# Jimmy2027/MoPoE-MIMIC

Measured on AMD Instinct MI355X. Metric: samples/sec, higher is better.
Workload: dtype f32; 1 GPU; BASELINE config c2: MoPoE joint-ELBO train step, 3 modalities (PA+Lateral+text) 128x128, class_dim 128, DIM_img 64, DIM_text 128, vocab 3517, batch 64/GPU, fp32 (storage, accumulation and every product; where the launch plan says so the fp32 products are formed on the bf16 matrix pipe from exact three-way splits of both operands -- closer to fp64 than the fp32 MFMA, tests: test_f32_products_on_the; global_batch=64, parallelism=dp1, hip_graph=True, cross_rank_elbo=mean

## Files before the change

### include/mopoe_hip.h

```cpp
#ifndef MOPOE_HIP_H
#define MOPOE_HIP_H

#include <stddef.h>
#include <stdint.h>

#ifdef __cplusplus
extern "C" {
#endif

#define MOPOE_ABI_VERSION 23

#define MOPOE_OK 0
#define MOPOE_ERR_ARG (-1)
#define MOPOE_ERR_LAUNCH (-2)
#define MOPOE_ERR_DEVICE (-3)

int mopoe_abi_version(void);
const char* mopoe_last_error(void);

typedef struct {
  int32_t N;
  int32_t Hs, Ws;
  int32_t Hb, Wb;
  int32_t Cin, Cout;
  int32_t kh, kw;
  int32_t sh, sw;
  int32_t ph, pw;
  int32_t transposed;
} mopoe_conv_geom;

typedef struct {
  const double* sums;
  const float* gamma;
  const float* beta;
  const float* rmean;
  const float* rvar;
  double inv_count;
  float eps;
  int32_t C;
  int32_t mode;
} mopoe_bn_ref;

typedef struct {
  const float* mask;
  int32_t kind;
  int32_t rows_per_sample;
} mopoe_mask_ref;

size_t mopoe_conv_workspace_bytes(void);

typedef struct {
  int32_t tile;
  int32_t split;
} mopoe_conv_plan;

int mopoe_conv_fwd(const float* x, const float* wp, const float* bias, float* y,
                   const mopoe_conv_geom* g, const mopoe_bn_ref* bn_in, const mopoe_mask_ref* mask,
                   double* out_stats, const mopoe_conv_plan* plan, void* workspace, size_t workspace_bytes,
                   void* stream);

typedef struct {
  const void* s;
  mopoe_bn_ref bn;
  float a, b;
} mopoe_mix_ref;
int mopoe_conv_fwd_mix(const float* x, const float* wp, const float* bias, float* y, const mopoe_conv_geom* g,
                       const mopoe_bn_ref* bn_in, const mopoe_mask_ref* mask, const mopoe_mix_ref* mix,
                       double* out_stats, const mopoe_conv_plan* plan, void* workspace, size_t workspace_bytes,
                       void* stream);

int mopoe_conv_dgrad(const float* dy, const float* wp, float* dx, const mopoe_conv_geom* g,
                     const mopoe_bn_ref* relu_bn, const float* xin, double* bwd_sums,
                     const mopoe_conv_plan* plan, void* workspace, size_t workspace_bytes, void* stream);

int mopoe_conv_wgrad(const float* x, const float* dy, float* dwp, const mopoe_conv_geom* g,
                     const mopoe_bn_ref* bn_in, int32_t dwp_is_zero, const mopoe_conv_plan* plan, void* stream);

int mopoe_block_out_fwd(const float* s, const float* m, float* out, int64_t rows, int32_t C,
                        const mopoe_bn_ref* bn_s, float a, float b, double* out_stats, void* stream);

int mopoe_bn_relu_apply(const float* x, float* out, int64_t rows, int32_t C, const mopoe_bn_ref* bn, void* stream);

int mopoe_bn_bwd_reduce(const float* g, const float* s, int64_t rows, int32_t C,
                        const mopoe_bn_ref* bn_s, double* sums, void* stream);

int mopoe_block_out_bwd(const float* g, const float* s, float* dm, float* ds, int64_t rows, int32_t C,
                        const mopoe_bn_ref* bn_s, const double* sums, const mopoe_mask_ref* mask,
                        float a, float b, float* dgamma, float* dbeta, float* colsum_dm,
                        float* colsum_ds, void* stream);

int mopoe_bn_bwd_apply(const float* dy, const float* x, const float* add, float* dx, int64_t rows,
                       int32_t C, const mopoe_bn_ref* bn, const double* sums,
                       const mopoe_mask_ref* mask, float* dgamma, float* dbeta, float* colsum_dx,
                       const float* next_s, const mopoe_bn_ref* next_bn, double* next_sums, void* stream);

typedef struct {
  const double* sums;
  float* rmean;
  float* rvar;
  int32_t C;
  int32_t count;
} mopoe_bn_running_desc;
int mopoe_bn_running_update(const mopoe_bn_running_desc* desc, int32_t n, float momentum, void* stream);

int mopoe_colsum(const float* x, float* out, int64_t rows, int32_t C, int32_t out_is_zero, void* stream);

int mopoe_latent_fwd(const float* const mu_in[3], const float* const lv_in[3], const float* eps,
                     int32_t B, int32_t D, const int32_t* row_start, const float* w, float norm,
                     float* mus, float* lvs, float* joint_mu, float* joint_lv, float* z, float* klds,
                     float* joint_div, double* kl_ws, void* stream);

int mopoe_latent_bwd(const float* const mu_in[3], const float* const lv_in[3], const float* eps,
                     int32_t B, int32_t D, const int32_t* row_start, const float* w, float norm,
                     const float* g_mus, const float* g_lvs, const float* g_joint_mu,
                     const float* g_joint_lv, const float* g_z, const float* g_klds,
                     const float* g_joint_div, float* const d_mu_in[3], float* const d_lv_in[3],
                     void* stream);

#define MOPOE_LATENT_MOE 0
#define MOPOE_LATENT_JSD 1
int mopoe_latent_mixture_fwd(int32_t method, const float* const mu_in[3], const float* const lv_in[3],
                             const float* eps, int32_t B, int32_t D, const int32_t* member_row_start,
                             const int32_t* comp_row_start, const float* w, float norm, float* sub_mu,
                             float* sub_lv, float* comp_mu, float* comp_lv, float* joint_mu, float* joint_lv,
                             float* z, float* klds, float* individual_divs, float* joint_div, float* pd_mu,
                             float* pd_lv, double* ws, void* stream);

int mopoe_latent_mixture_bwd(int32_t method, const float* const mu_in[3], const float* const lv_in[3],
                             const float* eps, int32_t B, int32_t D, const int32_t* member_row_start,
                             const int32_t* comp_row_start, const float* w, float norm, const float* g_sub_mu,
                             const float* g_sub_lv, const float* g_comp_mu, const float* g_comp_lv,
                             const float* g_joint_mu, const float* g_joint_lv, const float* g_z,
                             const float* g_klds, const float* g_individual_divs, const float* g_joint_div,
                             const float* g_pd_mu, const float* g_pd_lv, float* const d_mu_in[3],
                             float* const d_lv_in[3], void* stream);

int mopoe_latent_style_fwd(const float* const smu[3], const float* const slv[3], const float* const eps_s[3],
                           const int32_t S[3], int32_t B, int32_t D, const float* z, float norm, float* const zcat[3],
                           float* klds_style, double* ws, void* stream);

int mopoe_latent_style_bwd(const float* const smu[3], const float* const slv[3], const float* const eps_s[3],
                           const int32_t S[3], int32_t B, int32_t D, float norm, const float* const g_zcat[3],
                           const float* g_klds_style, float* const d_smu[3], float* const d_slv[3], float* g_z,
                           void* stream);

int mopoe_laplace_nll_fwd(const float* x_hat, const float* x, int64_t n, float scale, float norm,
                          float* out, double* ws, void* stream);
int mopoe_laplace_nll_bwd(const float* x_hat, const float* x, const float* g, int64_t n, float scale,
                          float norm, float* dx_hat, void* stream);

int mopoe_logsoftmax_fwd(const float* x, float* y, int64_t rows, int32_t V, void* stream);
int mopoe_logsoftmax_bwd(const float* dy, const float* y, float* dx, int64_t rows, int32_t V,
                         void* stream);
int mopoe_token_nll_fwd(const float* logp, const float* ids, int64_t rows, int32_t V, float norm,
                        float* out, double* ws, void* stream);
int mopoe_token_nll_bwd(const float* ids, const float* g, int64_t rows, int32_t V, float norm,
                        float* dlogp, void* stream);

int mopoe_dense_nll_fwd(const float* logp, const float* target, int64_t n, float norm, float* out, double* ws,
                        void* stream);
int mopoe_dense_nll_bwd(const float* target, const float* g, int64_t n, float norm, float* dlogp, void* stream);

int mopoe_laplace_logprob_rows(const float* x_hat, const float* x, int64_t rows, int64_t per_row,
// ... 104 lines not shown
```

### mopoe-mimic_amd/csrc/conv_gemm.hip

```cpp
#include "gemm_common.hpp"

namespace mopoe {

constexpr int BK = 16;
#ifndef TILE_N64_REMAINDER
#define TILE_N64_REMAINDER 64
#endif
#ifndef SPLIT_BLOCKS
#define SPLIT_BLOCKS 256
#endif
#ifndef SPLIT_TARGET
#define SPLIT_TARGET 512
#endif
#ifndef GEMM_8WAVES
#define GEMM_8WAVES 1
#endif
#ifndef PERSIST_BLOCKS
#define PERSIST_BLOCKS 2048
#endif
#ifndef GEMM_MIN_WAVES
#define GEMM_MIN_WAVES 3
#endif
#ifndef GEMM_BK_BIG
#define GEMM_BK_BIG 16
#endif
#ifndef GEMM_LDS_PAD
#define GEMM_LDS_PAD 4
#endif
constexpr int LDS_PAD = GEMM_LDS_PAD;

struct GemmArgs {
  const float* X;
  const float* W;
  float* Y;
  const float* bias;
  int N, Hx, Wx, Hy, Wy, Ck, Cn, Cin_w, Cout_w;
  int kh, kw, sh, sw, ph, pw;
  int form, w_nk;
  int Hq, Wq;
  long rows_per_phase;
  int vecA, vecB;
  mopoe_bn_ref bn_in;
  mopoe_mask_ref mask;
  double* out_stats;
  mopoe_bn_ref relu_bn;
  const float* xin;
  double* bwd_sums;
  unsigned x_bytes, w_bytes;
  int nsplit;
  float* partial;
  int* counters;
  long rows_total;
  int mix;
  float mix_a, mix_b;
  int xcd_remap;
};

__device__ __forceinline__ float epi_round(const GemmArgs&, float x) { return x; }
struct EpiXinRaw { float4 lo, hi; };
constexpr bool EPI_PREFETCH_XIN = false;
__device__ __forceinline__ EpiXinRaw epi_xin_ld(const GemmArgs& a, long yrow, int ncol, bool ok_hi) {
  const float* p = a.xin + yrow * a.Cn + ncol;
  EpiXinRaw r;
  r.lo = *reinterpret_cast<const float4*>(p);
  r.hi = ok_hi ? *reinterpret_cast<const float4*>(p + 4) : make_float4(0.f, 0.f, 0.f, 0.f);
  return r;
}
__device__ __forceinline__ void epi_xin_unpack(const EpiXinRaw& r, float (&xi)[8]) {
  xi[0] = r.lo.x; xi[1] = r.lo.y; xi[2] = r.lo.z; xi[3] = r.lo.w; xi[4] = r.hi.x; xi[5] = r.hi.y; xi[6] = r.hi.z; xi[7] = r.hi.w;
}
__device__ __forceinline__ void epi_store8(const GemmArgs& a, long yrow, int ncol, bool ok_hi, const float (&v)[8]) {
  float* dst = a.Y + yrow * a.Cn + ncol;
  *reinterpret_cast<float4*>(dst) = make_float4(v[0], v[1], v[2], v[3]);
  if (ok_hi) *reinterpret_cast<float4*>(dst + 4) = make_float4(v[4], v[5], v[6], v[7]);
}


__device__ __forceinline__ float4 bld4(__amdgpu_buffer_rsrc_t srd, unsigned byte_off) {
  const u32x4 v = __builtin_amdgcn_raw_buffer_load_b128(srd, byte_off, 0, 0);
  return make_float4(__uint_as_float(v.x), __uint_as_float(v.y), __uint_as_float(v.z), __uint_as_float(v.w));
}

__device__ __forceinline__ float4 bld4s(__amdgpu_buffer_rsrc_t srd, unsigned byte_off, unsigned s_off) {
  const u32x4 v = __builtin_amdgcn_raw_buffer_load_b128(srd, byte_off, s_off, 0);
  return make_float4(__uint_as_float(v.x), __uint_as_float(v.y), __uint_as_float(v.z), __uint_as_float(v.w));
}

__device__ __forceinline__ float4 ld4(const float* p, int nvalid, bool vec) {
  float4 v = make_float4(0.f, 0.f, 0.f, 0.f);
  if (nvalid >= 4 && vec) {
    v = *reinterpret_cast<const float4*>(p);
  } else {
    if (nvalid > 0) v.x = p[0];
    if (nvalid > 1) v.y = p[1];
    if (nvalid > 2) v.z = p[2];
    if (nvalid > 3) v.w = p[3];
  }
  return v;
}

template <int BM, int BN, int WGM, int WGN, int GBK, bool VEC, int SPEC = 0>
__global__ __launch_bounds__(64 * WGM * WGN, (WGM * WGN == 4 ? GEMM_MIN_WAVES : ((BM / WGM) * (BN / WGN) > 64 * 32 ? 2 : 4)))
void gather_gemm_kernel(const GemmArgs a) {
  static_assert(SPEC == 0 || VEC, "specialised loops exist for the vector path only");
  constexpr int NT = 64 * WGM * WGN;
  static_assert(WGM * WGN == 4 || WGM * WGN == 8, "4 or 8 waves per block");
  constexpr int WM = BM / WGM, WN = BN / WGN;
  constexpr int TI = WM / 32, TJ = WN / 32;
  constexpr int A_LD = BM + LDS_PAD, B_LD = BN + LDS_PAD;
  constexpr int KQ = GBK / 4;
  constexpr int RPP = NT / KQ;
  constexpr int A_PER_THR = BM / RPP;
  static_assert(BM % RPP == 0, "A tile rows must be a multiple of the rows covered per pass");
  constexpr int B_PER_THR_NK = (BN + RPP - 1) / RPP;
  constexpr int N4 = BN / 4;
  constexpr int B_PER_THR_KN = (GBK * N4 + NT - 1) / NT;
  constexpr int B_PER_THR = B_PER_THR_NK > B_PER_THR_KN ? B_PER_THR_NK : B_PER_THR_KN;

  constexpr int STG_LD = WN + 4;
  constexpr int A_FLOATS = 2 * GBK * A_LD, B_FLOATS = 2 * GBK * B_LD;
  constexpr int STG_FLOATS = VEC ? (NT / 64) * 32 * STG_LD : 0;
  constexpr int SMEM_FLOATS = (A_FLOATS + B_FLOATS) > STG_FLOATS ? (A_FLOATS + B_FLOATS) : STG_FLOATS;
  __shared__ __attribute__((aligned(16))) float smem[SMEM_FLOATS];
  __shared__ __attribute__((aligned(16))) float bnS[MAX_BN_C];
  __shared__ __attribute__((aligned(16))) float bnT[MAX_BN_C];
  __shared__ __attribute__((aligned(16))) float epi[5][VEC ? BN : 4];
  __shared__ int s_ticket;
  float* const As0 = smem;
  float* const Bs0 = smem + A_FLOATS;
#define AS_(buf, k, r) As0[((buf) * GBK + (k)) * A_LD + (r)]
#define BS_(buf, k, r) Bs0[((buf) * GBK + (k)) * B_LD + (r)]

  const int tid = threadIdx.x;
  const int lane = tid & 63, wave = tid >> 6;
  const int wm = wave / WGN, wn = wave % WGN;
  unsigned lbx = blockIdx.x, lby = blockIdx.y, lbz = blockIdx.z;
  if (a.xcd_remap) {
    const unsigned inner = gridDim.y * gridDim.z;
    const unsigned sw = xcd_swizzle(blockIdx.x + gridDim.x * (blockIdx.y + gridDim.y * blockIdx.z), gridDim.x * inner);
    lbx = sw / inner;
    const unsigned rem = sw - lbx * inner;
    lby = rem % gridDim.y;
    lbz = rem / gridDim.y;
  }
  const int n0 = lby * BN;
  const int phase = lbz / a.nsplit;
  const int split = lbz - phase * a.nsplit;

  const TapWalk tw = tap_walk(a, phase);
  const int nty = tw.nty, ntx = tw.ntx, ky0 = tw.ky0, kx0 = tw.kx0, kstep_y = tw.kstep_y, kstep_x = tw.kstep_x;
  const int dsgn = tw.dsgn, cy = tw.cy, cx = tw.cx, phy = tw.phy, phx = tw.phx;
  const int nkc = (a.Ck + GBK - 1) / GBK;
  const int total_all = nty * ntx * nkc;
// ... 359 lines not shown
  float cbias[TJ], s1[TJ], s2[TJ];
  BnC rbc[TJ];
  unsigned voffB[TJ];
#pragma unroll
  for (int j = 0; j < TJ; ++j) {
    const int n = n0 + wn * WN + j * 32 + l31;
    s1[j] = s2[j] = 0.f;
    cbias[j] = (n < a.Cn && a.bias && !a.partial) ? a.bias[n] : 0.f;
    rbc[j] = BnC{0.f, 0.f, 0.f, 0.f};
    if (n < a.Cn && do_relu_bn && !a.partial) rbc[j] = bn_coef(a.relu_bn, n);
    if (n < a.Cn) voffB[j] = w_nk ? ((unsigned)n * (unsigned)a.Cout_w + (unsigned)lhi * 4u) * 4u
                                  : ((unsigned)lhi * 4u * (unsigned)a.Cout_w + (unsigned)n) * 4u;
    else voffB[j] = OOB;
  }

  const long nMt = (a.rows_per_phase + BM - 1) / BM;
  for (long mt = lbx; mt < nMt; mt += gridDim.x) {
    const long m0 = mt * BM;
    int ry0[TI], rx0[TI], rbase[TI];
    bool rvalid[TI];
#pragma unroll
    for (int i = 0; i < TI; ++i) {
      const long m = m0 + wm * WM + i * 32 + l31;
      rvalid[i] = m < a.rows_per_phase;
      const unsigned mm = rvalid[i] ? (unsigned)m : 0u;
      const int n = (int)(mm / (unsigned)hw);
      const int rem = (int)(mm - (unsigned)n * (unsigned)hw);
      const int qy = rem / a.Wq, qx = rem - qy * a.Wq;
      if (a.form == 0) { ry0[i] = qy * a.sh - a.ph; rx0[i] = qx * a.sw - a.pw; }
      else             { ry0[i] = qy + cy;          rx0[i] = qx + cx; }
      rbase[i] = (n * a.Hx + ry0[i]) * a.Wx + rx0[i];
    }

    int ld_tap = it_beg / nkc;
    int ld_kc = (it_beg - ld_tap * nkc) * KS;
    bool tap_dirty = true;
    unsigned offA[TI], offW = 0;
    bool okA[TI];
    float4 ra[2][TI], rsc[2], rsh[2];
    float rbd[2][TJ][4];
    float4 rb4[2][TJ];
    bool rok[2][TI];

    auto load_step = [&](auto bufc) {
      constexpr int buf = decltype(bufc)::value;
      if (tap_dirty) {
        const int jy = ld_tap / ntx, jx = ld_tap - jy * ntx;
        const int wtap = (ky0 + kstep_y * jy) * a.kw + (kx0 + kstep_x * jx);
        const int tapoff = dsgn * (jy * a.Wx + jx);
#pragma unroll
        for (int i = 0; i < TI; ++i) {
          const int iy = ry0[i] + dsgn * jy, ix = rx0[i] + dsgn * jx;
          okA[i] = rvalid[i] & ((unsigned)iy < (unsigned)a.Hx) & ((unsigned)ix < (unsigned)a.Wx);
          offA[i] = okA[i] ? (unsigned)(rbase[i] + tapoff) * (unsigned)a.Ck * 4u + (unsigned)lhi * 16u : OOB;
        }
        offW = (unsigned)wtap * (unsigned)a.Cin_w * (unsigned)a.Cout_w * 4u;
        tap_dirty = false;
      }
      const unsigned sA = (unsigned)ld_kc * 4u;
#pragma unroll
      for (int i = 0; i < TI; ++i) { ra[buf][i] = bld4s(srdX, offA[i], sA); rok[buf][i] = okA[i]; }
      if (w_nk) {
        const unsigned sB = offW + (unsigned)ld_kc * 4u;
#pragma unroll
        for (int j = 0; j < TJ; ++j) rb4[buf][j] = bld4s(srdW, voffB[j], sB);
      } else {
#pragma unroll
        for (int e = 0; e < 4; ++e) {
          const unsigned sB = offW + (unsigned)(ld_kc + e) * (unsigned)a.Cout_w * 4u;
#pragma unroll
          for (int j = 0; j < TJ; ++j) rbd[buf][j][e] = bld1s(srdW, voffB[j], sB);
        }
      }
      if (xform) {
        rsc[buf] = *reinterpret_cast<const float4*>(&bnS[ld_kc + lhi * 4]);
        rsh[buf] = *reinterpret_cast<const float4*>(&bnT[ld_kc + lhi * 4]);
      }
      ld_kc += KS;
      if (ld_kc >= a.Ck) { ld_kc = 0; ++ld_tap; tap_dirty = true; }
    };

    f32x16 acc[TI][TJ];
#pragma unroll
    for (int i = 0; i < TI; ++i)
#pragma unroll
      for (int j = 0; j < TJ; ++j)
#pragma unroll
        for (int r = 0; r < 16; ++r) acc[i][j][r] = 0.f;

    auto mma_step = [&](auto bufc) {
      constexpr int buf = decltype(bufc)::value;
      float av[TI][4];
#pragma unroll
      for (int i = 0; i < TI; ++i) {
        float4 v = ra[buf][i];
        if (xform) {
          const bool ok = rok[buf][i];
          v.x = ok ? fmaxf(fmaf(v.x, rsc[buf].x, rsh[buf].x), 0.f) : 0.f;
          v.y = ok ? fmaxf(fmaf(v.y, rsc[buf].y, rsh[buf].y), 0.f) : 0.f;
          v.z = ok ? fmaxf(fmaf(v.z, rsc[buf].z, rsh[buf].z), 0.f) : 0.f;
          v.w = ok ? fmaxf(fmaf(v.w, rsc[buf].w, rsh[buf].w), 0.f) : 0.f;
        }
        av[i][0] = v.x; av[i][1] = v.y; av[i][2] = v.z; av[i][3] = v.w;
      }
#pragma unroll
      for (int e = 0; e < 4; ++e) {
#pragma unroll
        for (int j = 0; j < TJ; ++j) {
          float bv;
          if (w_nk) bv = e == 0 ? rb4[buf][j].x : (e == 1 ? rb4[buf][j].y : (e == 2 ? rb4[buf][j].z : rb4[buf][j].w));
          else bv = rbd[buf][j][e];
#pragma unroll
          for (int i = 0; i < TI; ++i)
            acc[i][j] = __builtin_amdgcn_mfma_f32_32x32x2f32(av[i][e], bv, acc[i][j], 0, 0, 0);
        }
      }
    };

    if (total > 0) load_step(std::integral_constant<int, 0>{});
    for (int it = 0; it < total; it += 2) {
      if (it + 1 < total) load_step(std::integral_constant<int, 1>{});
      __builtin_amdgcn_sched_barrier(0);
      mma_step(std::integral_constant<int, 0>{});
      if (it + 1 < total) {
        if (it + 2 < total) load_step(std::integral_constant<int, 0>{});
        __builtin_amdgcn_sched_barrier(0);
        mma_step(std::integral_constant<int, 1>{});
      }
    }

#include "gemm_epilogue.inc"
  }

#include "gemm_colstats.inc"
}

struct WgradArgs {
  const float* Xs;
  const float* Dy;
  float* dW;
  int N, Hs, Ws, Hb, Wb, Cin, Cout, kh, kw, sh, sw, ph, pw;
  int x_is_big;
  long Ms;
  long chunk;
  int nJ;
  int atomic;
  int vecI, vecJ;
  unsigned x_bytes, dy_bytes;
  int fast;
  mopoe_bn_ref bn_in;  int xcd_remap;
};

template <int BI, int BJ, bool VEC, int SPEC = 0>
__global__ __launch_bounds__(256) void wgrad_gemm_kernel(const WgradArgs a) {
  static_assert(SPEC == 0 || VEC, "specialised loops exist for the vector path only");
  constexpr int WI = BI / 2, WJ = BJ / 2;
  constexpr int TI = WI / 32, TJ = WJ / 32;
  constexpr int I_LD = BI + LDS_PAD, J_LD = BJ + LDS_PAD;
  constexpr int I4 = BI / 4, J4 = BJ / 4;
  constexpr int I_PER_THR = (BK * I4) / 256, J_PER_THR = (BK * J4) / 256;

  __shared__ __attribute__((aligned(16))) float Is[2][BK][I_LD];
  __shared__ __attribute__((aligned(16))) float Js[2][BK][J_LD];
  __shared__ __attribute__((aligned(16))) float bnS[MAX_BN_C];
  __shared__ __attribute__((aligned(16))) float bnT[MAX_BN_C];

  const int tid = threadIdx.x;
  const int lane = tid & 63, wave = tid >> 6;
  const int wi = wave >> 1, wj = wave & 1;
  const unsigned lin = a.xcd_remap ? xcd_swizzle(blockIdx.x + gridDim.x * (blockIdx.y + gridDim.y * blockIdx.z),
                                                 gridDim.x * gridDim.y * gridDim.z)
                                   : blockIdx.x + gridDim.x * (blockIdx.y + gridDim.y * blockIdx.z);
  const unsigned bx = lin % gridDim.x, byz = lin / gridDim.x;
  const unsigned by = byz % gridDim.y, bz = byz / gridDim.y;
  const int it_i = bx / a.nJ, it_j = bx % a.nJ;
  const int i0 = it_i * BI, j0 = it_j * BJ;
  const int tap = by;
  const int ky = tap / a.kw, kx = tap % a.kw;
  const long mbeg = (long)bz * a.chunk;
  const long mend = mbeg + a.chunk < a.Ms ? mbeg + a.chunk : a.Ms;
  const int total = (int)((mend - mbeg + BK - 1) / BK);

  const bool xform = SPEC ? (SPEC == 2) : (a.bn_in.mode != 0);
  const bool fast = SPEC ? true : (VEC && a.fast != 0);
  if (xform) {
    for (int c = tid; c < ((a.Cin + 3) & ~3); c += 256) {
      BnC k = BnC{0.f, 0.f, 0.f, 0.f};
      if (c < a.Cin) k = bn_coef(a.bn_in, c);
      bnS[c] = k.scale;
      bnT[c] = k.shift;
    }
    __syncthreads();
  }

  float4 ri[I_PER_THR], rj[J_PER_THR];
  bool pend_ok[I_PER_THR];
  const int hw = a.Hs * a.Ws;
  const __amdgpu_buffer_rsrc_t srdX = __builtin_amdgcn_make_buffer_rsrc((void*)a.Xs, 0, (int)a.x_bytes, 0x00020000);
  const __amdgpu_buffer_rsrc_t srdD = __builtin_amdgcn_make_buffer_rsrc((void*)a.Dy, 0, (int)a.dy_bytes, 0x00020000);

  static_assert(BI == BJ, "both operand tiles cover the same pixels per thread");
  constexpr int PPP = 256 / I4;
  int pn[I_PER_THR], pqy[I_PER_THR], pqx[I_PER_THR];
  long pm[I_PER_THR];
#pragma unroll
  for (int t = 0; t < I_PER_THR; ++t) {
    pm[t] = mbeg + tid / I4 + t * PPP;
    const unsigned m = (unsigned)(pm[t] < a.Ms ? pm[t] : 0);
    const unsigned n = m / (unsigned)hw;
    const unsigned rem = m - n * (unsigned)hw;
    pn[t] = (int)n; pqy[t] = rem / a.Ws; pqx[t] = rem - pqy[t] * a.Ws;
  }

  float4 sc4 = make_float4(0.f, 0.f, 0.f, 0.f), sh4 = sc4;
  const int ci = i0 + (tid % I4) * 4, cj = j0 + (tid % J4) * 4;
  if (xform) {
    const int cs = ci < a.Cin ? ci : 0;
    sc4 = *reinterpret_cast<const float4*>(&bnS[cs]);
    sh4 = *reinterpret_cast<const float4*>(&bnT[cs]);
  }

  const int rpc = a.Ws >= BK ? 1 : BK / a.Ws;
  const int big_c = a.x_is_big ? a.Cin : a.Cout;
  const unsigned shift_rows = (unsigned)(a.ph * a.Wb + a.pw);
  const unsigned shift_bytes = shift_rows * (unsigned)big_c * 4u;
  const __amdgpu_buffer_rsrc_t srdBig = __builtin_amdgcn_make_buffer_rsrc(
      (void*)((const char*)(a.x_is_big ? a.Xs : a.Dy) - shift_bytes), 0,
      (int)((a.x_is_big ? a.x_bytes : a.dy_bytes) + shift_bytes), 0x00020000);
  int f_ly[I_PER_THR], f_lx[I_PER_THR];
  unsigned f_vbig[I_PER_THR], f_vsmall_i[I_PER_THR], f_vsmall_j[I_PER_THR];
  int f_slot[I_PER_THR];
  int f_n = 0, f_qy = 0, f_qx = 0;
  unsigned f_m0 = 0;
  if (fast) {
#pragma unroll
    for (int t = 0; t < I_PER_THR; ++t) {
      const int p = tid / I4 + t * PPP;
      const int pdy = a.Ws >= BK ? 0 : p / a.Ws, pqx = a.Ws >= BK ? p : p - (p / a.Ws) * a.Ws;
      f_slot[t] = p;
      f_ly[t] = pdy * a.sh + ky - a.ph;
      f_lx[t] = pqx * a.sw + kx - a.pw;
      const unsigned lane_rows = (unsigned)((f_ly[t] + a.ph) * a.Wb + (f_lx[t] + a.pw));
      const int cbig = a.x_is_big ? ci : cj;
      f_vbig[t] = (cbig < big_c) ? (lane_rows * (unsigned)big_c + (unsigned)cbig) * 4u : OOB;
      f_vsmall_i[t] = (ci < a.Cin) ? ((unsigned)p * (unsigned)a.Cin + (unsigned)ci) * 4u : OOB;
      f_vsmall_j[t] = (cj < a.Cout) ? ((unsigned)p * (unsigned)a.Cout + (unsigned)cj) * 4u : OOB;
    }
    const unsigned m0 = (unsigned)mbeg;
    f_m0 = m0;
    f_n = (int)(m0 / (unsigned)hw);
    const unsigned rem = m0 - (unsigned)f_n * (unsigned)hw;
    f_qy = (int)(rem / (unsigned)a.Ws);
    f_qx = (int)(rem - (unsigned)f_qy * (unsigned)a.Ws);
  }

  auto load_tiles = [&](int ) {
    if (fast) {
      if constexpr (VEC) {
        const int nleft = (int)((unsigned)mend - f_m0);
        const int s_by = f_qy * a.sh, s_bx = f_qx * a.sw;
        const unsigned s_big = (unsigned)((f_n * a.Hb + s_by) * a.Wb + s_bx) * (unsigned)big_c * 4u;
        const unsigned s_small_i = f_m0 * (unsigned)a.Cin * 4u, s_small_j = f_m0 * (unsigned)a.Cout * 4u;
#pragma unroll
        for (int t = 0; t < I_PER_THR; ++t) {
          const bool inm = f_slot[t] < nleft;
          const bool inb = ((unsigned)(s_by + f_ly[t]) < (unsigned)a.Hb) & ((unsigned)(s_bx + f_lx[t]) < (unsigned)a.Wb);
          const unsigned vb = (inm & inb) ? f_vbig[t] : OOB;
          if (a.x_is_big) {
            ri[t] = bld4s(srdBig, vb, s_big);
            rj[t] = bld4s(srdD, inm ? f_vsmall_j[t] : OOB, s_small_j);
            pend_ok[t] = (inm & inb) & (ci < a.Cin);
          } else {
            ri[t] = bld4s(srdX, inm ? f_vsmall_i[t] : OOB, s_small_i);
            rj[t] = bld4s(srdBig, vb, s_big);
            pend_ok[t] = inm & (ci < a.Cin);
          }
        }
        f_m0 += BK;
        if (a.Ws >= BK) { f_qx += BK; if (f_qx >= a.Ws) { f_qx = 0; ++f_qy; } }
        else f_qy += rpc;
        if (f_qy >= a.Hs) { f_qy = 0; ++f_n; }
      }
      return;
    }
#pragma unroll
    for (int t = 0; t < I_PER_THR; ++t) {
      const bool inm = pm[t] < mend;
      const int by = pqy[t] * a.sh - a.ph + ky, bx = pqx[t] * a.sw - a.pw + kx;
      const bool inb = ((unsigned)by < (unsigned)a.Hb) & ((unsigned)bx < (unsigned)a.Wb);
      const int srow = (int)pm[t];
      const int brow = (pn[t] * a.Hb + by) * a.Wb + bx;
      const int rowx = a.x_is_big ? brow : srow, rowd = a.x_is_big ? srow : brow;
      const bool okx = inm & (ci < a.Cin) & (a.x_is_big ? inb : true);
      const bool okd = inm & (cj < a.Cout) & (a.x_is_big ? true : inb);
      pend_ok[t] = okx;
      if constexpr (VEC) {
        ri[t] = bld4(srdX, okx ? ((unsigned)rowx * (unsigned)a.Cin + (unsigned)ci) * 4u : OOB);
        rj[t] = bld4(srdD, okd ? ((unsigned)rowd * (unsigned)a.Cout + (unsigned)cj) * 4u : OOB);
      } else {
        float4 v = make_float4(0.f, 0.f, 0.f, 0.f), w = v;
        if (okx) v = ld4(a.Xs + (long)rowx * a.Cin + ci, a.Cin - ci, false);
        if (okd) w = ld4(a.Dy + (long)rowd * a.Cout + cj, a.Cout - cj, false);
        ri[t] = v; rj[t] = w;
      }
      pm[t] += BK;
      pqx[t] += BK;
      if (pqx[t] >= a.Ws) {
        if (a.Ws >= BK) {
          pqx[t] -= a.Ws; ++pqy[t];
        } else {
          const int carry = pqx[t] / a.Ws;
          pqx[t] -= carry * a.Ws; pqy[t] += carry;
        }
        if (pqy[t] >= a.Hs) {
          const int carry = pqy[t] / a.Hs;
          pqy[t] -= carry * a.Hs; pn[t] += carry;
        }
      }
    }
  };

  auto store_tiles = [&](auto bufc) {
    constexpr int buf = decltype(bufc)::value;
#pragma unroll
    for (int t = 0; t < I_PER_THR; ++t) {
      const int p = tid / I4 + t * (256 / I4);
      if (xform) {
        const bool ok = pend_ok[t];
        ri[t].x = ok ? fmaxf(fmaf(ri[t].x, sc4.x, sh4.x), 0.f) : 0.f;
        ri[t].y = ok ? fmaxf(fmaf(ri[t].y, sc4.y, sh4.y), 0.f) : 0.f;
        ri[t].z = ok ? fmaxf(fmaf(ri[t].z, sc4.z, sh4.z), 0.f) : 0.f;
        ri[t].w = ok ? fmaxf(fmaf(ri[t].w, sc4.w, sh4.w), 0.f) : 0.f;
      }
      *reinterpret_cast<float4*>(&Is[buf][p][(tid % I4) * 4]) = ri[t];
    }
#pragma unroll
    for (int t = 0; t < J_PER_THR; ++t) {
      const int p = tid / J4 + t * (256 / J4);
      *reinterpret_cast<float4*>(&Js[buf][p][(tid % J4) * 4]) = rj[t];
    }
  };

  f32x16 acc[TI][TJ];
#pragma unroll
  for (int i = 0; i < TI; ++i)
#pragma unroll
    for (int j = 0; j < TJ; ++j)
#pragma unroll
      for (int r = 0; r < 16; ++r) acc[i][j][r] = 0.f;

  if (total > 0) {
    load_tiles(0);
    store_tiles(std::integral_constant<int, 0>{});
  }
  __syncthreads();

  const int l31 = lane & 31, lhi = lane >> 5;
  auto chunk = [&](int it, auto curc) {
    constexpr int cur = decltype(curc)::value;
    if (it + 1 < total) load_tiles(it + 1);
    __builtin_amdgcn_sched_barrier(0);
#pragma unroll
    for (int kk = 0; kk < BK / 2; ++kk) {
      const int k = kk * 2 + lhi;
      float av[TI], bv[TJ];
#pragma unroll
      for (int i = 0; i < TI; ++i) av[i] = Is[cur][k][wi * WI + i * 32 + l31];
#pragma unroll
      for (int j = 0; j < TJ; ++j) bv[j] = Js[cur][k][wj * WJ + j * 32 + l31];
#pragma unroll
      for (int i = 0; i < TI; ++i)
#pragma unroll
        for (int j = 0; j < TJ; ++j)
          acc[i][j] = __builtin_amdgcn_mfma_f32_32x32x2f32(av[i], bv[j], acc[i][j], 0, 0, 0);
    }
    if (it + 1 < total) store_tiles(std::integral_constant<int, cur ^ 1>{});
    __syncthreads();
  };
  int it = 0;
  for (; it + 1 < total; it += 2) {
    chunk(it, std::integral_constant<int, 0>{});
    chunk(it + 1, std::integral_constant<int, 1>{});
  }
  if (it < total) chunk(it, std::integral_constant<int, 0>{});

#pragma unroll
  for (int j = 0; j < TJ; ++j) {
    const int co = j0 + wj * WJ + j * 32 + l31;
    if (co >= a.Cout) continue;
#pragma unroll
    for (int i = 0; i < TI; ++i) {
#pragma unroll
      for (int r = 0; r < 16; ++r) {
        const int ci = i0 + wi * WI + i * 32 + (r & 3) + 8 * (r >> 2) + 4 * lhi;
        if (ci >= a.Cin) continue;
        float* dst = a.dW + ((long)tap * a.Cin + ci) * a.Cout + co;
        if (a.atomic) unsafeAtomicAdd(dst, acc[i][j][r]);
        else *dst = acc[i][j][r];
      }
    }
  }
}

#ifndef EPI_MAX_BLOCKS_Y
#define EPI_MAX_BLOCKS_Y 256
#endif
__global__ __launch_bounds__(256) void splitk_epilogue_kernel(const GemmArgs a) {
  __shared__ float cs[2][4][64];
  const int tx = threadIdx.x & 63, ty = threadIdx.x >> 6;
  const int n = blockIdx.x * 64 + tx;
  const bool nok = n < a.Cn;
  const bool do_relu_bn = a.relu_bn.mode != 0;
  const float bias = (nok && a.bias) ? a.bias[n] : 0.f;
  BnC rb = {0.f, 0.f, 0.f, 0.f};
  if (nok && do_relu_bn) rb = bn_coef(a.relu_bn, n);
  const long stride = a.rows_total * (long)a.Cn;
  float s1 = 0.f, s2 = 0.f;
  if (nok) {
    for (long row = (long)blockIdx.y * 4 + ty; row < a.rows_total; row += (long)gridDim.y * 4) {
      const float* p = a.partial + row * a.Cn + n;
      float acc8[8] = {0.f, 0.f, 0.f, 0.f, 0.f, 0.f, 0.f, 0.f};
      int s = 0;
      for (; s + 8 <= a.nsplit; s += 8) {
#pragma unroll
        for (int u = 0; u < 8; ++u) acc8[u] += p[(long)(s + u) * stride];
      }
      for (; s < a.nsplit; ++s) acc8[s & 7] += p[(long)s * stride];
      float x = bias + (((acc8[0] + acc8[1]) + (acc8[2] + acc8[3])) + ((acc8[4] + acc8[5]) + (acc8[6] + acc8[7])));
      if (a.mask.kind != 0) x *= mask_at(a.mask, row, n, a.Cn);
      if (do_relu_bn) {
        const float xi = a.xin[row * a.Cn + n];
        x = (fmaf(xi, rb.scale, rb.shift) > 0.f) ? x : 0.f;
        s1 += x;
        s2 += x * ((xi - rb.mean) * rb.rstd);
      } else {
        s1 += x;
        s2 += x * x;
      }
      a.Y[row * a.Cn + n] = x;
    }
  }
  double* sums = do_relu_bn ? a.bwd_sums : a.out_stats;
  if (sums) {
    cs[0][ty][tx] = s1;
    cs[1][ty][tx] = s2;
    __syncthreads();
    if (ty == 0 && nok) {
      atomic_add_f64(sums + n, (double)((cs[0][0][tx] + cs[0][1][tx]) + (cs[0][2][tx] + cs[0][3][tx])));
      atomic_add_f64(sums + a.Cn + n, (double)((cs[1][0][tx] + cs[1][1][tx]) + (cs[1][2][tx] + cs[1][3][tx])));
    }
  }
}


#include "gemm_glds_common.inc"
#include "conv_gemm_glds.inc"
#include "conv_gemm_glds_parity.inc"


static int launch_gather(const float* X, const float* W, const float* bias, float* Y, const mopoe_conv_geom* g,
                         int dest_on_small, int Ck, int Cn, int w_nk, const mopoe_bn_ref* bn_in,
                         const mopoe_mask_ref* mask, double* out_stats, const mopoe_bn_ref* relu_bn,
                         const float* xin, double* bwd_sums, const mopoe_conv_plan* plan, void* ws, size_t ws_bytes,
                         hipStream_t stream, const mopoe_mix_ref* mix = nullptr) {
  int* counters = nullptr;
  if (ws && ws_bytes > WS_COUNTER_BYTES) { counters = (int*)ws; ws = (char*)ws + WS_COUNTER_BYTES; ws_bytes -= WS_COUNTER_BYTES; }
  else { ws = nullptr; ws_bytes = 0; }
  GemmArgs a;
  a.X = X; a.W = W; a.Y = Y; a.bias = bias;
  a.N = g->N; a.Ck = Ck; a.Cn = Cn; a.Cin_w = g->Cin; a.Cout_w = g->Cout;
  a.kh = g->kh; a.kw = g->kw; a.sh = g->sh; a.sw = g->sw; a.ph = g->ph; a.pw = g->pw;
  a.w_nk = w_nk;
  int nphase;
  if (dest_on_small) {
    a.form = 0; a.Hx = g->Hb; a.Wx = g->Wb; a.Hy = g->Hs; a.Wy = g->Ws; a.Hq = g->Hs; a.Wq = g->Ws; nphase = 1;
  } else {
    a.form = 1; a.Hx = g->Hs; a.Wx = g->Ws; a.Hy = g->Hb; a.Wy = g->Wb; a.Hq = g->Hb / g->sh; a.Wq = g->Wb / g->sw;
    nphase = g->sh * g->sw;
  }
  a.rows_per_phase = (long)g->N * a.Hq * a.Wq;
  a.rows_total = (long)g->N * a.Hy * a.Wy;
  a.vecA = (Ck % 4 == 0) && aligned16(X);
  a.vecB = (g->Cout % 4 == 0) && aligned16(W);
  const size_t xb = (size_t)g->N * a.Hx * a.Wx * Ck * sizeof(float);
  const size_t wb = (size_t)g->kh * g->kw * g->Cin * g->Cout * sizeof(float);
  const bool vec = a.vecA && a.vecB && xb < (1ull << 31) && wb < (1ull << 31) && Cn % 4 == 0 && aligned16(Y) &&
                   (!xin || aligned16(xin)) && (!mask || mask->kind == 0 || aligned16(mask->mask));
  a.x_bytes = (unsigned)std::min<size_t>(xb, 0x7fffffffu);
  a.w_bytes = (unsigned)std::min<size_t>(wb, 0x7fffffffu);
  mopoe_bn_ref none = {};
  mopoe_mask_ref nomask = {nullptr, 0, 1};
  a.bn_in = bn_in ? *bn_in : none;
  a.mask = mask ? *mask : nomask;
  a.out_stats = out_stats;
  a.relu_bn = relu_bn ? *relu_bn : none;
  a.xin = xin; a.bwd_sums = bwd_sums;
  a.mix = 0; a.mix_a = a.mix_b = 0.f;
  static const bool xcd_remap_g = !getenv("MOPOE_NO_XCD_REMAP");
  a.xcd_remap = xcd_remap_g ? 1 : 0;
  if (mix) {
    if (!mix->s || mix->bn.mode == 0 || relu_bn || xin) { set_error("conv_fwd_mix: needs s and its BatchNorm"); return MOPOE_ERR_ARG; }
    if (!vec || !aligned16(mix->s)) { set_error("conv_fwd_mix: channel counts must be multiples of 4 and tensors 16-byte aligned"); return MOPOE_ERR_ARG; }
    a.mix = 1; a.mix_a = mix->a; a.mix_b = mix->b;
    a.relu_bn = mix->bn; a.xin = (const float*)mix->s;
  }
  a.nsplit = 1; a.partial = nullptr; a.counters = nullptr;
  static const bool dbg_nostats = getenv("MOPOE_DEBUG_NOSTATS") != nullptr;
  if (dbg_nostats) { a.out_stats = nullptr; a.bwd_sums = nullptr; }
  if (a.bn_in.mode != 0 && (a.bn_in.C != Ck || Ck > MAX_BN_C)) { set_error("bn_in channel mismatch (%d vs %d)", a.bn_in.C, Ck); return MOPOE_ERR_ARG; }
  if (a.relu_bn.mode != 0 && (a.relu_bn.C != Cn || !a.xin)) { set_error("relu_bn needs xin and C == %d", Cn); return MOPOE_ERR_ARG; }
  if (a.mask.kind != 0 && !a.mask.mask) { set_error("mask pointer missing"); return MOPOE_ERR_ARG; }
  if (a.mask.kind == 1 && a.mask.rows_per_sample != a.Hy * a.Wy) { set_error("channel mask: rows_per_sample must be Hout*Wout"); return MOPOE_ERR_ARG; }
  if (a.rows_total >= (1L << 31) || (long)g->N * a.Hx * a.Wx >= (1L << 31)) { set_error("conv: more than 2^31 rows"); return MOPOE_ERR_ARG; }

  int cfg;
  bool emu = false;
  if (Cn > 64) cfg = (a.rows_per_phase > 64 || Cn >= 256) ? 0 : 2;
  else cfg = a.rows_per_phase >= 256L * 64 ? 1 : 2;
#ifdef TILE_N64_REMAINDER
  if (cfg == 0 && (Cn % 128) == 64 && a.rows_per_phase >= 256L * TILE_N64_REMAINDER) cfg = 1;
#endif
  if (plan && plan->tile >= 0) {
    if (plan->tile > 19) { set_error("conv plan: tile %d (see mopoe_conv_plan in mopoe_hip.h: 0..19)", plan->tile); return MOPOE_ERR_ARG; }
    cfg = plan->tile;
    if (cfg >= 16) {
      if (a.bn_in.mode != 0) { set_error("conv plan: tile %d (split-bf16 products) has no BN-on-load form", cfg); return MOPOE_ERR_ARG; }
      emu = true;
      cfg -= 4;
    }
    if (cfg >= 12 && (!vec || Ck % 32 != 0 || (a.bn_in.mode != 0 && cfg == 13))) {
      set_error("conv plan: tile %d (LDS-DMA family) needs the vector path, K channels %% 32 == 0 (Ck = %d) and, with BN on load, tile 12, 14 or 15", cfg, Ck);
      return MOPOE_ERR_ARG;
    }
    if (cfg >= 3 && !vec) cfg = cfg == 3 ? 0 : 2;
    if ((cfg == 5 || cfg == 6) && Ck % 32 != 0) cfg -= 3;
    if (cfg >= 8 && cfg < 12 && (!vec || Ck % 8 != 0 || a.mix)) cfg = (cfg == 8) ? 0 : (cfg == 9 ? 1 : (cfg == 10 ? 2 : 4));
  }
  static const int TILE_BM[16] = {128, 256, 64, 256, 128, 64, 128, 128, 128, 256, 64, 128, 128, 128, 64, 256};
  static const int TILE_BN[16] = {128, 64, 64, 128, 64, 64, 64, 128, 128, 64, 64, 64, 128, 64, 64, 128};
  const int bm = TILE_BM[cfg], bn = TILE_BN[cfg];
  const long nMt = ceil_div(a.rows_per_phase, bm);
  const int nNt = ceil_div(Cn, bn);
  const int gbk = (cfg == 5 || cfg == 6 || cfg >= 12) ? 32 : (cfg >= 8 ? 8 : 16);
  const int nkc = ceil_div(Ck, gbk);
  const int iters = (dest_on_small ? g->kh * g->kw : std::max(1, (g->kh / g->sh) * (g->kw / g->sw))) * nkc;
  const long blocks = nMt * nNt * nphase;
  const size_t per = (size_t)a.rows_total * Cn * sizeof(float);
  if (plan && plan->split > 0) {
    long ns = std::min<long>(plan->split, iters);
    if (ns >= 2 && (!ws || (size_t)ns * per > ws_bytes)) {
      set_error("conv plan: split %ld needs %zu workspace bytes (have %zu)", ns, (size_t)ns * per, ws ? ws_bytes : (size_t)0);
      return MOPOE_ERR_ARG;
    }
    if (ns >= 2) { a.nsplit = (int)ns; a.partial = (float*)ws; }
  } else if (ws && blocks < SPLIT_BLOCKS && iters * gbk >= 256) {
    long ns = std::min<long>((SPLIT_TARGET + blocks - 1) / blocks, (long)iters * gbk / 128);
    if ((size_t)ns * per > ws_bytes) ns = (long)(ws_bytes / per);
    if (ns >= 2) { a.nsplit = (int)ns; a.partial = (float*)ws; }
  }
  const bool in_kernel_reduce = vec && (cfg < 8 || cfg >= 12);
  if (a.partial && in_kernel_reduce) {
    if (blocks > (long)(WS_COUNTER_BYTES / sizeof(int))) { set_error("conv: split reduction over %ld output tiles (at most %zu)", blocks, WS_COUNTER_BYTES / sizeof(int)); return MOPOE_ERR_ARG; }
    a.counters = counters;
  }
  const long persist = cfg >= 12 ? (cfg == 15 ? 256 : 512)
                                 : (cfg >= 8 ? 4096 : ((cfg == 2 || cfg >= 4) ? PERSIST_BLOCKS * 3 / 2 : PERSIST_BLOCKS));
  long gx = std::min<long>(nMt, std::max<long>(1, persist / ((long)nNt * nphase * a.nsplit)));
  double taps_eff = dest_on_small ? (double)g->kh * g->kw : (double)g->kh * g->kw / ((double)g->sh * g->sw);
  const double flops = 2.0 * (double)g->N * a.Hy * a.Wy * (double)Cn * (double)Ck * taps_eff;
  {
    const int spec = (vec && Ck % gbk == 0) ? (w_nk ? 3 : (a.bn_in.mode != 0 ? 2 : 1)) : 0;
    const double abytes = ((double)g->N * a.Hx * a.Wx * Ck + (double)a.rows_total * Cn) * sizeof(float);
    ProfScope prof(stream, flops, emu ? PROF_F32_GLDS_EMU + (cfg - 12) * 2 + (spec == 3 ? 1 : 0)
                                      : cfg >= 12 ? PROF_F32_GLDS + (cfg - 12) * 3 + (spec - 1)
                                            : (cfg >= 8 ? PROF_DIRECT + (cfg - 8) * 4 + spec
                                                        : (vec ? PROF_GATHER_VEC + cfg * 4 + spec : PROF_GATHER_SCALAR + cfg)), abytes);
    dim3 grid((unsigned)gx, nNt, nphase * a.nsplit);
#define MOPOE_LAUNCH_TILE(BM_, BN_, WM_, WN_, BK_, THREADS_)                                                                    \
  do {                                                                                                                          \
    if (spec == 1) hipLaunchKernelGGL((gather_gemm_kernel<BM_, BN_, WM_, WN_, BK_, true, 1>), grid, dim3(THREADS_), 0, stream, a);      \
    else if (spec == 2) hipLaunchKernelGGL((gather_gemm_kernel<BM_, BN_, WM_, WN_, BK_, true, 2>), grid, dim3(THREADS_), 0, stream, a); \
    else if (spec == 3) hipLaunchKernelGGL((gather_gemm_kernel<BM_, BN_, WM_, WN_, BK_, true, 3>), grid, dim3(THREADS_), 0, stream, a); \
    else hipLaunchKernelGGL((gather_gemm_kernel<BM_, BN_, WM_, WN_, 16, true, 0>), grid, dim3(THREADS_), 0, stream, a);                \
  } while (0)
#define MOPOE_LAUNCH_DIRECT(WM_, WN_, TI_, TJ_)                                                                                   \
  do {                                                                                                                          \
    if (spec == 1) hipLaunchKernelGGL((direct_gemm_kernel<WM_, WN_, TI_, TJ_, 1>), grid, dim3(64 * WM_ * WN_), 0, stream, a);      \
    else if (spec == 2) hipLaunchKernelGGL((direct_gemm_kernel<WM_, WN_, TI_, TJ_, 2>), grid, dim3(64 * WM_ * WN_), 0, stream, a); \
    else hipLaunchKernelGGL((direct_gemm_kernel<WM_, WN_, TI_, TJ_, 3>), grid, dim3(64 * WM_ * WN_), 0, stream, a);                \
  } while (0)
#define MOPOE_LAUNCH_GLDS(BM_, BN_, WM_, WN_, ST_)                                                                                       \
  do {                                                                                                                                \
    if (spec == 1) hipLaunchKernelGGL((gather_gemm_f32_glds_kernel<BM_, BN_, WM_, WN_, 1, ST_>), grid, dim3(64 * WM_ * WN_), 0, stream, a); \
    else hipLaunchKernelGGL((gather_gemm_f32_glds_kernel<BM_, BN_, WM_, WN_, 3, ST_>), grid, dim3(64 * WM_ * WN_), 0, stream, a);          \
  } while (0)
#define MOPOE_LAUNCH_GLDS_EMU(BM_, BN_, WM_, WN_, ST_)                                                                                   \
  do {                                                                                                                                \
    if (spec == 1) hipLaunchKernelGGL((gather_gemm_f32_glds_kernel<BM_, BN_, WM_, WN_, 1, ST_, 1>), grid, dim3(64 * WM_ * WN_), 0, stream, a); \
    else hipLaunchKernelGGL((gather_gemm_f32_glds_kernel<BM_, BN_, WM_, WN_, 3, ST_, 1>), grid, dim3(64 * WM_ * WN_), 0, stream, a);          \
  } while (0)
    if (emu) {
      if (cfg == 12) MOPOE_LAUNCH_GLDS_EMU(128, 128, 2, 2, 2);
      else if (cfg == 13) MOPOE_LAUNCH_GLDS_EMU(128, 64, 2, 2, 3);
      else if (cfg == 14) MOPOE_LAUNCH_GLDS_EMU(64, 64, 2, 2, 4);
      else MOPOE_LAUNCH_GLDS_EMU(256, 128, 4, 2, 3);
    }
#undef MOPOE_LAUNCH_GLDS_EMU
    else if (cfg >= 12) {
      if (spec == 2) {
        if (cfg == 12) hipLaunchKernelGGL((gather_gemm_f32_glds_kernel<128, 128, 2, 2, 2, 2>), grid, dim3(256), 0, stream, a);
        else if (cfg == 14) hipLaunchKernelGGL((gather_gemm_f32_glds_kernel<64, 64, 2, 2, 2, 4>), grid, dim3(256), 0, stream, a);
        else hipLaunchKernelGGL((gather_gemm_f32_glds_kernel<256, 128, 4, 2, 2, 2>), grid, dim3(512), 0, stream, a);
      }
      else if (cfg == 12) MOPOE_LAUNCH_GLDS(128, 128, 2, 2, 2);
      else if (cfg == 13) MOPOE_LAUNCH_GLDS(128, 64, 2, 2, 3);
      else if (cfg == 14) MOPOE_LAUNCH_GLDS(64, 64, 2, 2, 4);
      else MOPOE_LAUNCH_GLDS(256, 128, 4, 2, 2);
    }
#undef MOPOE_LAUNCH_GLDS
    else if (cfg == 8) MOPOE_LAUNCH_DIRECT(2, 2, 2, 2);
    else if (cfg == 9) MOPOE_LAUNCH_DIRECT(4, 1, 2, 2);
    else if (cfg == 10) MOPOE_LAUNCH_DIRECT(2, 2, 1, 1);
    else if (cfg == 11) MOPOE_LAUNCH_DIRECT(2, 1, 2, 2);
    else if (vec) {
      if (cfg == 0) MOPOE_LAUNCH_TILE(128, 128, 2, 4, 16, 512);
      else if (cfg == 1) MOPOE_LAUNCH_TILE(256, 64, 4, 2, 16, 512);
      else if (cfg == 3) MOPOE_LAUNCH_TILE(256, 128, 4, 2, 16, 512);
      else if (cfg == 4) MOPOE_LAUNCH_TILE(128, 64, 2, 2, 16, 256);
      else if (cfg == 5) MOPOE_LAUNCH_TILE(64, 64, 2, 2, 32, 256);
      else if (cfg == 6) MOPOE_LAUNCH_TILE(128, 64, 2, 2, 32, 256);
      else if (cfg == 7) MOPOE_LAUNCH_TILE(128, 128, 2, 2, 16, 256);
      else MOPOE_LAUNCH_TILE(64, 64, 2, 2, 16, 256);
    } else {
      if (cfg == 0) hipLaunchKernelGGL((gather_gemm_kernel<128, 128, 2, 2, GEMM_BK_BIG, false>), grid, dim3(256), 0, stream, a);
      else if (cfg == 1) hipLaunchKernelGGL((gather_gemm_kernel<256, 64, 4, 1, 16, false>), grid, dim3(256), 0, stream, a);
      else hipLaunchKernelGGL((gather_gemm_kernel<64, 64, 2, 2, 16, false>), grid, dim3(256), 0, stream, a);
    }
#undef MOPOE_LAUNCH_TILE
#undef MOPOE_LAUNCH_DIRECT
    if (int rc = check_launch("gather_gemm")) return rc;
    if (a.partial && !in_kernel_reduce) {
      dim3 eg(ceil_div(Cn, 64), std::min<long>(ceil_div(a.rows_total, 4), EPI_MAX_BLOCKS_Y));
      hipLaunchKernelGGL(splitk_epilogue_kernel, eg, dim3(256), 0, stream, a);
      if (int rc = check_launch("splitk_epilogue")) return rc;
    }
  }
  return MOPOE_OK;
}

}

using namespace mopoe;

extern "C" size_t mopoe_conv_workspace_bytes(void) { return WS_RECOMMENDED; }

extern "C" int mopoe_conv_fwd(const float* x, const float* wp, const float* bias, float* y, const mopoe_conv_geom* g,
                              const mopoe_bn_ref* bn_in, const mopoe_mask_ref* mask, double* out_stats,
                              const mopoe_conv_plan* plan, void* workspace, size_t workspace_bytes, void* stream) {
  if (int rc = validate_geom(g)) return rc;
  if (!x || !wp || !y) { set_error("conv_fwd: null pointer"); return MOPOE_ERR_ARG; }
  const bool plain = (!bn_in || bn_in->mode == 0) && (!mask || mask->kind == 0);
  if (plain && !g->transposed && g->Cin == 1 && !bias && edge_supported(g, g->Cout, {wp, y}))
    return edge_expand(x, wp, y, g, g->Cout, out_stats, (hipStream_t)stream);
  if (plain && g->transposed && g->Cout == 1 && !out_stats && edge_supported(g, g->Cin, {x, wp}))
    return edge_reduce(x, wp, bias, y, g, g->Cin, (hipStream_t)stream);
  return launch_gather(x, wp, bias, y, g, g->transposed ? 0 : 1, g->Cin, g->Cout, 0, bn_in, mask, out_stats,
                       nullptr, nullptr, nullptr, plan, workspace, workspace_bytes, (hipStream_t)stream);
}

extern "C" int mopoe_conv_fwd_mix(const float* x, const float* wp, const float* bias, float* y, const mopoe_conv_geom* g,
                                  const mopoe_bn_ref* bn_in, const mopoe_mask_ref* mask, const mopoe_mix_ref* mix,
                                  double* out_stats, const mopoe_conv_plan* plan, void* workspace, size_t workspace_bytes,
                                  void* stream) {
  if (int rc = validate_geom(g)) return rc;
  if (!x || !wp || !y || !mix) { set_error("conv_fwd_mix: null pointer"); return MOPOE_ERR_ARG; }
  return launch_gather(x, wp, bias, y, g, g->transposed ? 0 : 1, g->Cin, g->Cout, 0, bn_in, mask, out_stats,
                       nullptr, nullptr, nullptr, plan, workspace, workspace_bytes, (hipStream_t)stream, mix);
}

extern "C" int mopoe_conv_dgrad(const float* dy, const float* wp, float* dx, const mopoe_conv_geom* g,
                                const mopoe_bn_ref* relu_bn, const float* xin, double* bwd_sums,
                                const mopoe_conv_plan* plan, void* workspace, size_t workspace_bytes, void* stream) {
  if (int rc = validate_geom(g)) return rc;
  if (!dy || !wp || !dx) { set_error("conv_dgrad: null pointer"); return MOPOE_ERR_ARG; }
  if (g->transposed && g->Cout == 1 && (!relu_bn || relu_bn->mode == 0) && edge_supported(g, g->Cin, {wp, dx}))
    return edge_expand(dy, wp, dx, g, g->Cin, nullptr, (hipStream_t)stream);
  return launch_gather(dy, wp, nullptr, dx, g, g->transposed ? 1 : 0, g->Cout, g->Cin, 1, nullptr, nullptr,
                       nullptr, relu_bn, xin, bwd_sums, plan, workspace, workspace_bytes, (hipStream_t)stream);
}

extern "C" int mopoe_conv_wgrad(const float* x, const float* dy, float* dwp, const mopoe_conv_geom* g,
                                const mopoe_bn_ref* bn_in, int32_t dwp_is_zero, const mopoe_conv_plan* plan,
                                void* stream_) {
  if (int rc = validate_geom(g)) return rc;
  if (!x || !dy || !dwp) { set_error("conv_wgrad: null pointer"); return MOPOE_ERR_ARG; }
  hipStream_t stream = (hipStream_t)stream_;
  if ((!bn_in || bn_in->mode == 0) && !g->transposed && g->Cin == 1 && edge_supported(g, g->Cout, {dy, dwp}))
    return edge_wgrad(dy, x, dwp, g, g->Cout, stream, dwp_is_zero != 0);
  if ((!bn_in || bn_in->mode == 0) && g->transposed && g->Cout == 1 && edge_supported(g, g->Cin, {x, dwp}))
    return edge_wgrad(x, dy, dwp, g, g->Cin, stream, dwp_is_zero != 0);
  WgradArgs a;
  a.Xs = x; a.Dy = dy; a.dW = dwp;
  a.N = g->N; a.Hs = g->Hs; a.Ws = g->Ws; a.Hb = g->Hb; a.Wb = g->Wb; a.Cin = g->Cin; a.Cout = g->Cout;
  a.kh = g->kh; a.kw = g->kw; a.sh = g->sh; a.sw = g->sw; a.ph = g->ph; a.pw = g->pw;
  a.x_is_big = g->transposed ? 0 : 1;
  a.Ms = (long)g->N * g->Hs * g->Ws;
  mopoe_bn_ref none = {};
  a.bn_in = bn_in ? *bn_in : none;
  if (a.bn_in.mode != 0 && (a.bn_in.C != g->Cin || g->Cin > MAX_BN_C)) { set_error("wgrad bn_in channel mismatch"); return MOPOE_ERR_ARG; }
  a.vecI = (g->Cin % 4 == 0) && aligned16(x);
  a.vecJ = (g->Cout % 4 == 0) && aligned16(dy);
  const size_t rows_x = (size_t)g->N * (g->transposed ? g->Hs * g->Ws : g->Hb * g->Wb);
  const size_t rows_dy = (size_t)g->N * (g->transposed ? g->Hb * g->Wb : g->Hs * g->Ws);
  const size_t xb = rows_x * g->Cin * sizeof(float), db = rows_dy * g->Cout * sizeof(float);
  const bool vec = a.vecI && a.vecJ && xb < (1ull << 31) && db < (1ull << 31);
  a.x_bytes = (unsigned)std::min<size_t>(xb, 0x7fffffffu);
  a.dy_bytes = (unsigned)std::min<size_t>(db, 0x7fffffffu);
  if (rows_x >= (1ull << 31) || rows_dy >= (1ull << 31)) { set_error("wgrad: more than 2^31 rows"); return MOPOE_ERR_ARG; }
  const int hw_s = g->Hs * g->Ws;
  a.fast = (vec && ((g->Ws % BK == 0) || (BK % g->Ws == 0 && hw_s % BK == 0))) ? 1 : 0;
  const int taps = g->kh * g->kw;
  bool big = g->Cin > 64 && g->Cout > 64;
  if (plan && (plan->tile == 9 || plan->tile == 10)) {
    const bool ok = a.bn_in.mode == 0 && vec && g->kh == 4 && g->kw == 4 && g->sh == 2 && g->sw == 2 && g->ph == 1 && g->pw == 1 &&
                    g->Hs % 8 == 0 && g->Ws % 8 == 0 && g->Hb == 2 * g->Hs && g->Wb == 2 * g->Ws;
    if (!ok) {
      set_error("wgrad plan: tiles 9 / 10 (four taps per block) need a plain operand, the vector path, k4 s2 p1 and a small grid of whole 8 x 8 tiles");
      return MOPOE_ERR_ARG;
    }
    const int Cg = a.x_is_big ? g->Cin : g->Cout, Csm = a.x_is_big ? g->Cout : g->Cin;
    const int cs = plan->tile == 10 ? 128 : 64;
    if (cs == 128 && Csm % 128 != 0) { set_error("wgrad plan: tile 10 needs a multiple of 128 channels on the small-grid operand (%d)", Csm); return MOPOE_ERR_ARG; }
    const long ntiles = (long)g->N * (g->Hs / 8) * (g->Ws / 8);
    const long cblocks = (long)ceil_div(Cg, 64) * ceil_div(Csm, cs) * 4;
    long split = plan->split > 0 ? plan->split : (256 + cblocks - 1) / cblocks;
    if (split > ntiles) split = ntiles;
    if (split < 1) split = 1;
    a.chunk = (ntiles + split - 1) / split;
    split = (ntiles + a.chunk - 1) / a.chunk;
    a.atomic = split > 1;
    static const bool xcd_remap9 = !getenv("MOPOE_NO_XCD_REMAP");
    a.xcd_remap = xcd_remap9 ? 1 : 0;
    if (a.atomic && !dwp_is_zero) {
      if (hipMemsetAsync(dwp, 0, (size_t)taps * g->Cin * g->Cout * sizeof(float), stream) != hipSuccess) { set_error("wgrad memset failed"); return MOPOE_ERR_LAUNCH; }
    }
    ProfScope prof(stream, 2.0 * (double)a.Ms * g->Cin * (double)g->Cout * taps, PROF_F32_WGRAD_PARITY + (cs == 128 ? 2 : 0) + (a.x_is_big ? 0 : 1), (double)xb + (double)db);
    const dim3 grid((unsigned)(ceil_div(Cg, 64) * ceil_div(Csm, cs)), 4, (unsigned)split);
    if (cs == 128 && a.x_is_big) hipLaunchKernelGGL((wgrad_parity_f32_kernel<128, true>), grid, dim3(256), 0, stream, a);
    else if (cs == 128) hipLaunchKernelGGL((wgrad_parity_f32_kernel<128, false>), grid, dim3(256), 0, stream, a);
    else if (a.x_is_big) hipLaunchKernelGGL((wgrad_parity_f32_kernel<64, true>), grid, dim3(256), 0, stream, a);
    else hipLaunchKernelGGL((wgrad_parity_f32_kernel<64, false>), grid, dim3(256), 0, stream, a);
    return check_launch("wgrad_parity_f32 (four taps per block)");
  }
  const bool wemu = plan && (plan->tile == 7 || plan->tile == 8);
  if (wemu && a.bn_in.mode != 0) { set_error("wgrad plan: tile %d (split-bf16 products) has no BN-on-load form", plan->tile); return MOPOE_ERR_ARG; }
  if (plan && (plan->tile == 2 || plan->tile == 6 || plan->tile == 8)) big = false;
  else if (plan && (plan->tile == 5 || plan->tile == 7)) {
    if (!big) { set_error("wgrad plan: tile %d (128x128 on LDS-DMA) needs more than 64 channels on both sides (%d, %d)", plan->tile, g->Cin, g->Cout); return MOPOE_ERR_ARG; }
  }
  else if (plan && plan->tile > 2) { set_error("wgrad plan: tile %d (see mopoe_conv_plan in mopoe_hip.h: -1, 0, 2, 5, 6, 7, 8, 9, 10)", plan->tile); return MOPOE_ERR_ARG; }
  const bool glds = plan && plan->tile >= 5;
  if (glds && !vec) { set_error("wgrad plan: the LDS-DMA tiles need the vector path (channel counts %% 4 == 0, aligned tensors)"); return MOPOE_ERR_ARG; }
  const int T = big ? 128 : 64;
  const int nI = ceil_div(g->Cin, T), nJ = ceil_div(g->Cout, T);
  a.nJ = nJ;
  const long tiles = (long)nI * nJ * taps;
  long split = (1024 + tiles - 1) / tiles;
  if (plan && plan->split > 0) split = plan->split;
  const int kp = glds ? 32 : BK;
  const long max_split = glds ? (a.Ms + 4 * kp - 1) / (4 * kp) : (a.Ms + 8 * BK - 1) / (8 * BK);
  if (split > max_split) split = max_split;
  if (split < 1) split = 1;
  long chunk = (a.Ms + split - 1) / split;
  chunk = (chunk + kp - 1) / kp * kp;
  split = (a.Ms + chunk - 1) / chunk;
  a.chunk = chunk;
  a.atomic = split > 1;
  static const bool xcd_remap = !getenv("MOPOE_NO_XCD_REMAP");
  a.xcd_remap = xcd_remap ? 1 : 0;
  const size_t bytes = (size_t)taps * g->Cin * g->Cout * sizeof(float);
  if (a.atomic && !dwp_is_zero) {
    if (hipMemsetAsync(dwp, 0, bytes, stream) != hipSuccess) { set_error("wgrad memset failed"); return MOPOE_ERR_LAUNCH; }
  }
  const double flops = 2.0 * (double)a.Ms * g->Cin * (double)g->Cout * taps;
  const int spec = a.fast ? (a.bn_in.mode != 0 ? 2 : 1) : 0;
  const double abytes = ((double)g->N * g->Hs * g->Ws * (g->transposed ? g->Cin : g->Cout)
                         + (double)g->N * g->Hb * g->Wb * (g->transposed ? g->Cout : g->Cin)) * sizeof(float);
  ProfScope prof(stream, flops, wemu ? PROF_F32_WGRAD_GLDS_EMU + (big ? 0 : 1)
                                : glds ? PROF_F32_WGRAD_GLDS + (big ? 0 : 2) + (a.bn_in.mode != 0 ? 1 : 0)
                                     : (vec ? PROF_WGRAD_VEC + (big ? 0 : 3) + spec : PROF_WGRAD_SCALAR + (big ? 0 : 1)), abytes);
  dim3 grid(nI * nJ, taps, (unsigned)split);
  if (wemu) {
    if (big) hipLaunchKernelGGL((wgrad_gemm_f32_glds_kernel<128, false, 2, 1>), grid, dim3(256), 0, stream, a);
    else hipLaunchKernelGGL((wgrad_gemm_f32_glds_kernel<64, false, 4, 1>), grid, dim3(256), 0, stream, a);
  } else if (glds) {
    const bool xf = a.bn_in.mode != 0;
    if (big) {
      if (xf) hipLaunchKernelGGL((wgrad_gemm_f32_glds_kernel<128, true, 2>), grid, dim3(256), 0, stream, a);
      else hipLaunchKernelGGL((wgrad_gemm_f32_glds_kernel<128, false, 2>), grid, dim3(256), 0, stream, a);
    } else {
      if (xf) hipLaunchKernelGGL((wgrad_gemm_f32_glds_kernel<64, true, 2>), grid, dim3(256), 0, stream, a);
      else hipLaunchKernelGGL((wgrad_gemm_f32_glds_kernel<64, false, 4>), grid, dim3(256), 0, stream, a);
    }
  } else if (vec) {
    if (big) {
      if (spec == 1) hipLaunchKernelGGL((wgrad_gemm_kernel<128, 128, true, 1>), grid, dim3(256), 0, stream, a);
      else if (spec == 2) hipLaunchKernelGGL((wgrad_gemm_kernel<128, 128, true, 2>), grid, dim3(256), 0, stream, a);
      else hipLaunchKernelGGL((wgrad_gemm_kernel<128, 128, true, 0>), grid, dim3(256), 0, stream, a);
    } else {
      if (spec == 1) hipLaunchKernelGGL((wgrad_gemm_kernel<64, 64, true, 1>), grid, dim3(256), 0, stream, a);
      else if (spec == 2) hipLaunchKernelGGL((wgrad_gemm_kernel<64, 64, true, 2>), grid, dim3(256), 0, stream, a);
      else hipLaunchKernelGGL((wgrad_gemm_kernel<64, 64, true, 0>), grid, dim3(256), 0, stream, a);
    }
  } else {
    if (big) hipLaunchKernelGGL((wgrad_gemm_kernel<128, 128, false>), grid, dim3(256), 0, stream, a);
    else hipLaunchKernelGGL((wgrad_gemm_kernel<64, 64, false>), grid, dim3(256), 0, stream, a);
  }
  return check_launch("wgrad_gemm");
}
```

### mopoe-mimic_amd/csrc/conv_gemm_glds.inc

```
typedef float f32x4v __attribute__((ext_vector_type(4)));

template <int OFF>
__device__ __forceinline__ void lds_frag_f4(f32x4v& r, unsigned addr) {
  static_assert(OFF >= 0 && OFF < 65536, "ds offset field");
  MOPOE_DEVICE_ASM("ds_read_b128 %0, %1 offset:%2" : "=v"(r) : "v"(addr), "n"(OFF) : "memory");
}
template <int OFF>
__device__ __forceinline__ void lds_frag_f1(float& r, unsigned addr) {
  static_assert(OFF >= 0 && OFF < 65536, "ds offset field");
  MOPOE_DEVICE_ASM("ds_read_b32 %0, %1 offset:%2" : "=v"(r) : "v"(addr), "n"(OFF) : "memory");
}

typedef __bf16 e_bf16x2 __attribute__((ext_vector_type(2)));
typedef __bf16 e_bf16x8 __attribute__((ext_vector_type(8)));
typedef float e_f32x2 __attribute__((ext_vector_type(2)));
struct Split3 { u32x4 h, m, l; };

__device__ __forceinline__ void split3_pair(float a0, float a1, unsigned& h, unsigned& m, unsigned& l) {
#if defined(MOPOE_DBG_EMU_NOSPLIT)
  h = __float_as_uint(a0); m = __float_as_uint(a1); l = h;
  return;
#endif
  const e_f32x2 a = {a0, a1};
  h = __builtin_bit_cast(unsigned, __builtin_convertvector(a, e_bf16x2));
// ... 278 lines not shown
#pragma unroll
      for (int i = 0; i < B_INSTR; ++i) lds_dma16(srdW, stage + A_BYTES + (i * NW + wave) * 1024, voffB[i], sB_set[set]);
    };

    f32x16 acc[TI][TJ];
#pragma unroll
    for (int i = 0; i < TI; ++i)
#pragma unroll
      for (int j = 0; j < TJ; ++j)
#pragma unroll
        for (int r = 0; r < 16; ++r) acc[i][j][r] = 0.f;

    using I0 = std::integral_constant<int, 0>; using I1 = std::integral_constant<int, 1>;
    using I2 = std::integral_constant<int, 2>; using I3 = std::integral_constant<int, 3>;
    if constexpr (xform) {
      if (total > 0) issue(I0{});
      if constexpr (R == 2) { if (total > 1) issue(I1{}); }
      if (total > 0) commit(I0{}, I0{});
      if (total > R) issue(I0{});
      if constexpr (NSTAGE == 4) {
        if (total > 1) commit(I1{}, I1{});
        if (total > 1 + R) issue(I1{});
        if (total > 2) commit(I2{}, I0{});
        if (total > 2 + R) issue(I0{});
      }
    } else {
      if (total > 0) issue(I0{});
      if (NSTAGE >= 3 && total > 1) issue(I1{});
      if (NSTAGE >= 4 && total > 2) issue(I2{});
    }

    auto chunk = [&](int it, auto curc) {
      constexpr int cur = decltype(curc)::value;
      if constexpr (xform) {
        if (R == 2 && it + NSTAGE - 2 + R < total) wait_vmcnt<LPS>();
        else wait_vmcnt<0>();
        asm volatile("s_waitcnt lgkmcnt(0)" ::: "memory");
      } else {
        const int younger = total - 1 - it < NSTAGE - 2 ? total - 1 - it : NSTAGE - 2;
        if (NSTAGE >= 4 && younger == 2) wait_vmcnt<2 * LPS>();
        else if (NSTAGE >= 3 && younger == 1) wait_vmcnt<LPS>();
        else wait_vmcnt<0>();
      }
      __builtin_amdgcn_sched_barrier(0);
      __builtin_amdgcn_s_barrier();
      __builtin_amdgcn_sched_barrier(0);
      if constexpr (xform) {
        constexpr int cbuf = (cur + NSTAGE - 1) % NSTAGE, cset = (cur + NSTAGE - 1) % R;
        if (it + NSTAGE - 1 < total) commit(std::integral_constant<int, cbuf>{}, std::integral_constant<int, cset>{});
        if (it + NSTAGE - 1 + R < total) issue(std::integral_constant<int, cset>{});
        __builtin_amdgcn_sched_barrier(0);
      } else {
        if (it + NSTAGE - 1 < total) issue(std::integral_constant<int, (cur + NSTAGE - 1) % NSTAGE>{});
      }
      constexpr unsigned stage_off = (unsigned)(cur * STAGE_BYTES);
      f32x4v fa[2][TI], fb[2][w_nk ? TJ : 1];
      float fk[2][w_nk ? 1 : TJ][4];
      auto read_step = [&](auto qc, auto setc) {
        constexpr int q = decltype(qc)::value, set = decltype(setc)::value;
#pragma unroll
        for (int i = 0; i < TI; ++i) lds_frag_f4<0>(fa[set][i], lds_base + stage_off + aoff[i][q]);
        if constexpr (w_nk) {
#pragma unroll
          for (int j = 0; j < TJ; ++j) lds_frag_f4<0>(fb[set][j], lds_base + stage_off + boff[j][w_nk ? q : 0]);
        } else {
#pragma unroll
          for (int j = 0; j < TJ; ++j) {
            lds_frag_f1<(8 * q + 0) * B_ROWB>(fk[set][j][0], lds_base + stage_off + boff[j][0]);
            lds_frag_f1<(8 * q + 1) * B_ROWB>(fk[set][j][1], lds_base + stage_off + boff[j][0]);
            lds_frag_f1<(8 * q + 2) * B_ROWB>(fk[set][j][2], lds_base + stage_off + boff[j][0]);
            lds_frag_f1<(8 * q + 3) * B_ROWB>(fk[set][j][3], lds_base + stage_off + boff[j][0]);
          }
        }
      };
      auto fence = [&](auto setc) {
        constexpr int set = decltype(setc)::value;
        if constexpr (w_nk) {
          if constexpr (TI == 2 && TJ == 2) MOPOE_DEVICE_ASM("s_waitcnt lgkmcnt(0)" : "+v"(fa[set][0]), "+v"(fa[set][1]), "+v"(fb[set][0]), "+v"(fb[set][1]) :: "memory");
          else if constexpr (TI == 2) MOPOE_DEVICE_ASM("s_waitcnt lgkmcnt(0)" : "+v"(fa[set][0]), "+v"(fa[set][1]), "+v"(fb[set][0]) :: "memory");
          else if constexpr (TJ == 2) MOPOE_DEVICE_ASM("s_waitcnt lgkmcnt(0)" : "+v"(fa[set][0]), "+v"(fb[set][0]), "+v"(fb[set][1]) :: "memory");
          else MOPOE_DEVICE_ASM("s_waitcnt lgkmcnt(0)" : "+v"(fa[set][0]), "+v"(fb[set][0]) :: "memory");
        } else {
          if constexpr (TI == 2 && TJ == 2)
            MOPOE_DEVICE_ASM("s_waitcnt lgkmcnt(0)" : "+v"(fa[set][0]), "+v"(fa[set][1]), "+v"(fk[set][0][0]), "+v"(fk[set][0][1]), "+v"(fk[set][0][2]),
                             "+v"(fk[set][0][3]), "+v"(fk[set][1][0]), "+v"(fk[set][1][1]), "+v"(fk[set][1][2]), "+v"(fk[set][1][3]) :: "memory");
          else if constexpr (TI == 2)
            MOPOE_DEVICE_ASM("s_waitcnt lgkmcnt(0)" : "+v"(fa[set][0]), "+v"(fa[set][1]), "+v"(fk[set][0][0]), "+v"(fk[set][0][1]), "+v"(fk[set][0][2]),
                             "+v"(fk[set][0][3]) :: "memory");
          else if constexpr (TJ == 2)
            MOPOE_DEVICE_ASM("s_waitcnt lgkmcnt(0)" : "+v"(fa[set][0]), "+v"(fk[set][0][0]), "+v"(fk[set][0][1]), "+v"(fk[set][0][2]),
                             "+v"(fk[set][0][3]), "+v"(fk[set][1][0]), "+v"(fk[set][1][1]), "+v"(fk[set][1][2]), "+v"(fk[set][1][3]) :: "memory");
          else
            MOPOE_DEVICE_ASM("s_waitcnt lgkmcnt(0)" : "+v"(fa[set][0]), "+v"(fk[set][0][0]), "+v"(fk[set][0][1]), "+v"(fk[set][0][2]),
                             "+v"(fk[set][0][3]) :: "memory");
        }
        __builtin_amdgcn_sched_barrier(0);
      };
      auto mfma_step = [&](auto setc) {
        constexpr int set = decltype(setc)::value;
#pragma unroll
        for (int e = 0; e < 4; ++e)
#pragma unroll
          for (int j = 0; j < TJ; ++j) {
            const float b = w_nk ? fb[set][w_nk ? j : 0][e] : fk[set][w_nk ? 0 : j][e];
#pragma unroll
            for (int i = 0; i < TI; ++i)
              acc[i][j] = __builtin_amdgcn_mfma_f32_32x32x2f32(fa[set][i][e], b, acc[i][j], 0, 0, 0);
          }
      };
      using I0 = std::integral_constant<int, 0>; using I1 = std::integral_constant<int, 1>;
      using I2 = std::integral_constant<int, 2>; using I3 = std::integral_constant<int, 3>;
      read_step(I0{}, I0{});
      fence(I0{});
      read_step(I1{}, I1{});
      mfma_step(I0{});
      fence(I1{});
      read_step(I2{}, I0{});
      mfma_step(I1{});
      fence(I0{});
      read_step(I3{}, I1{});
      mfma_step(I0{});
      fence(I1{});
      mfma_step(I1{});
      __builtin_amdgcn_sched_barrier(0);
    };
    if constexpr (EMU != 0) {
#include "conv_gemm_glds_emu.inc"
    } else {
      int it = 0;
      while (it < total) {
        chunk(it, std::integral_constant<int, 0>{});
        if (++it >= total) break;
        chunk(it, std::integral_constant<int, 1>{});
        if (++it >= total) break;
        if (NSTAGE >= 3) {
          chunk(it, std::integral_constant<int, 2 % NSTAGE>{});
          if (++it >= total) break;
        }
        if (NSTAGE >= 4) {
          chunk(it, std::integral_constant<int, 3 % NSTAGE>{});
          ++it;
        }
      }
    }
    __syncthreads();

#include "gemm_epilogue_rows.inc"
  }

#include "gemm_colstats_rows.inc"
}

template <int BI, bool XFORM, int NSTAGE, int EMU = 0>
__global__ __launch_bounds__(256, 2) void wgrad_gemm_f32_glds_kernel(const WgradArgs a) {
  static_assert(EMU == 0 || !XFORM, "EMU: plain operand form");
  constexpr int BJ = BI;
  constexpr int WI = BI / 2, WJ = BJ / 2, TI = WI / 32, TJ = WJ / 32;
  constexpr int KP = 32;
  constexpr int ROWB = BI * 4;
  static_assert(BI == 64 || BI == 128, "tiles of 64 or 128 channels");
  static_assert(NSTAGE >= 2 && NSTAGE <= 4 && (!XFORM || NSTAGE == 2), "two to four LDS buffers (two with BN on load)");
  constexpr int LPR = ROWB / 16, RPP = 64 / LPR;
  constexpr int IMG_BYTES = KP * ROWB;
  constexpr int STAGE_BYTES = 2 * IMG_BYTES;
  constexpr int NINSTR = IMG_BYTES / (256 * 16);
  static_assert(IMG_BYTES % (256 * 16) == 0 && NINSTR >= 1, "whole pieces");
  constexpr int LPS = 2 * NINSTR;
  constexpr int OFF_BN = NSTAGE * STAGE_BYTES;
  __shared__ __attribute__((aligned(1024))) unsigned char smem[OFF_BN + (XFORM ? 2 * MAX_BN_C * 4 : 16)];
  float* const bnS = reinterpret_cast<float*>(smem + OFF_BN);
  float* const bnT = bnS + MAX_BN_C;

  const int tid = threadIdx.x;
  const int lane = tid & 63, wave = __builtin_amdgcn_readfirstlane(tid >> 6);
  const int wi = wave >> 1, wj = wave & 1;
  const unsigned lin = a.xcd_remap ? xcd_swizzle(blockIdx.x + gridDim.x * (blockIdx.y + gridDim.y * blockIdx.z),
                                                 gridDim.x * gridDim.y * gridDim.z)
                                   : blockIdx.x + gridDim.x * (blockIdx.y + gridDim.y * blockIdx.z);
  const unsigned bx = lin % gridDim.x, byz = lin / gridDim.x;
  const unsigned by = byz % gridDim.y, bz = byz / gridDim.y;
  const int it_i = bx / a.nJ, it_j = bx % a.nJ;
  const int i0 = it_i * BI, j0 = it_j * BJ;
  const int tap = by;
  const int ky = tap / a.kw, kx = tap % a.kw;
  const long mbeg = (long)bz * a.chunk;
  const long mend = mbeg + a.chunk < a.Ms ? mbeg + a.chunk : a.Ms;
  const int total = (int)((mend - mbeg + KP - 1) / KP);

  if (XFORM) {
    for (int c = tid; c < ((a.Cin + 3) & ~3); c += 256) {
      BnC k = BnC{0.f, 0.f, 0.f, 0.f};
      if (c < a.Cin) k = bn_coef(a.bn_in, c);
      bnS[c] = k.scale;
      bnT[c] = k.shift;
    }
    __syncthreads();
  }
  const __amdgpu_buffer_rsrc_t srdX = __builtin_amdgcn_make_buffer_rsrc((void*)a.Xs, 0, (int)a.x_bytes, 0x00020000);
  const __amdgpu_buffer_rsrc_t srdD = __builtin_amdgcn_make_buffer_rsrc((void*)a.Dy, 0, (int)a.dy_bytes, 0x00020000);
  const unsigned lds_base = (unsigned)(uintptr_t)((lds_void_t*)smem);

  const int slot_in_piece = lane / LPR;
  const int ci = i0 + (lane % LPR) * 4, cj = j0 + (lane % LPR) * 4;
  const bool ci_ok = ci < a.Cin, cj_ok = cj < a.Cout;
  float4 sc = make_float4(0.f, 0.f, 0.f, 0.f), sh = sc;
  if (XFORM && ci_ok) {
    sc = *reinterpret_cast<const float4*>(&bnS[ci]);
    sh = *reinterpret_cast<const float4*>(&bnT[ci]);
  }
  const unsigned hw = (unsigned)(a.Hs * a.Ws);

  unsigned ioff[TI], joff[TJ];
  {
    const int l31 = lane & 31, lhi = lane >> 5;
#pragma unroll
    for (int i = 0; i < TI; ++i) ioff[i] = (unsigned)(4 * lhi) * (unsigned)ROWB + (unsigned)(wi * WI + i * 32 + l31) * 4u;
#pragma unroll
    for (int j = 0; j < TJ; ++j) joff[j] = (unsigned)IMG_BYTES + (unsigned)(4 * lhi) * (unsigned)ROWB + (unsigned)(wj * WJ + j * 32 + l31) * 4u;
  }

  float4 ri[XFORM ? NINSTR : 1];
  bool okx_reg[XFORM ? NINSTR : 1];
  unsigned offd_pending[XFORM ? NINSTR : 1];
  unsigned m_next = (unsigned)mbeg;

  auto offsets = [&](unsigned (&offx)[NINSTR], unsigned (&offd)[NINSTR], bool (&okx)[NINSTR]) {
#pragma unroll
    for (int t = 0; t < NINSTR; ++t) {
      const unsigned m = m_next + (unsigned)(RPP * (t * 4 + wave) + slot_in_piece);
      const bool inm = (long)m < mend;
      const unsigned n = m / hw;
      const unsigned rem = m - n * hw;
      const unsigned qy = rem / (unsigned)a.Ws, qx = rem - qy * (unsigned)a.Ws;
      const int yb = (int)qy * a.sh - a.ph + ky, xb = (int)qx * a.sw - a.pw + kx;
      const bool inb = ((unsigned)yb < (unsigned)a.Hb) & ((unsigned)xb < (unsigned)a.Wb);
      const unsigned brow = (n * (unsigned)a.Hb + (unsigned)yb) * (unsigned)a.Wb + (unsigned)xb;
      const unsigned rowx = a.x_is_big ? brow : m, rowd = a.x_is_big ? m : brow;
      okx[t] = inm & ci_ok & (a.x_is_big ? inb : true);
      const bool okd = inm & cj_ok & (a.x_is_big ? true : inb);
      offx[t] = okx[t] ? (rowx * (unsigned)a.Cin + (unsigned)ci) * 4u : OOB;
      offd[t] = okd ? (rowd * (unsigned)a.Cout + (unsigned)cj) * 4u : OOB;
    }
    m_next += KP;
  };
  auto issue = [&](auto bufc) {
    constexpr int buf = decltype(bufc)::value;
    unsigned offx[NINSTR], offd[NINSTR];
    bool okx[NINSTR];
    offsets(offx, offd, okx);
    unsigned char* const stage = smem + buf * STAGE_BYTES;
    if constexpr (XFORM) {
#pragma unroll
      for (int t = 0; t < NINSTR; ++t) { ri[t] = bld4(srdX, offx[t]); okx_reg[t] = okx[t]; offd_pending[t] = offd[t]; }
    } else {
#pragma unroll
      for (int t = 0; t < NINSTR; ++t) lds_dma16(srdX, stage + (t * 4 + wave) * 1024, offx[t], 0u);
#pragma unroll
      for (int t = 0; t < NINSTR; ++t) lds_dma16(srdD, stage + IMG_BYTES + (t * 4 + wave) * 1024, offd[t], 0u);
    }
  };
  auto commit = [&](auto bufc) {
    constexpr int buf = decltype(bufc)::value;
    unsigned char* const stage = smem + buf * STAGE_BYTES;
#pragma unroll
    for (int t = 0; t < NINSTR; ++t) {
      const float4 v = ri[XFORM ? t : 0];
      float4 o;
      o.x = fmaxf(fmaf(v.x, sc.x, sh.x), 0.f); o.y = fmaxf(fmaf(v.y, sc.y, sh.y), 0.f);
      o.z = fmaxf(fmaf(v.z, sc.z, sh.z), 0.f); o.w = fmaxf(fmaf(v.w, sc.w, sh.w), 0.f);
      if (!okx_reg[XFORM ? t : 0]) o = make_float4(0.f, 0.f, 0.f, 0.f);
      lds_store_b128(lds_base + (unsigned)(buf * STAGE_BYTES + (t * 4 + wave) * 1024) + (unsigned)lane * 16u, __builtin_bit_cast(u32x4, o));
    }
#pragma unroll
    for (int t = 0; t < NINSTR; ++t) lds_dma16(srdD, stage + IMG_BYTES + (t * 4 + wave) * 1024, offd_pending[XFORM ? t : 0], 0u);
  };

  f32x16 acc[TI][TJ];
#pragma unroll
  for (int i = 0; i < TI; ++i)
#pragma unroll
    for (int j = 0; j < TJ; ++j)
#pragma unroll
      for (int r = 0; r < 16; ++r) acc[i][j][r] = 0.f;

  if (total > 0) issue(std::integral_constant<int, 0>{});
  if constexpr (XFORM) {
    if (total > 0) commit(std::integral_constant<int, 0>{});
    if (total > 1) issue(std::integral_constant<int, 1>{});
  } else {
    if (NSTAGE >= 3 && total > 1) issue(std::integral_constant<int, 1>{});
    if (NSTAGE >= 4 && total > 2) issue(std::integral_constant<int, 2>{});
  }

  auto chunk = [&](int it, auto curc) {
    constexpr int cur = decltype(curc)::value;
    const int younger = total - 1 - it < NSTAGE - 2 ? total - 1 - it : NSTAGE - 2;
    if (NSTAGE >= 4 && younger == 2) wait_vmcnt<2 * LPS>();
    else if (NSTAGE >= 3 && younger == 1) wait_vmcnt<LPS>();
    else wait_vmcnt<0>();
    if constexpr (XFORM) asm volatile("s_waitcnt lgkmcnt(0)" ::: "memory");
    __builtin_amdgcn_sched_barrier(0);
    __builtin_amdgcn_s_barrier();
    __builtin_amdgcn_sched_barrier(0);
    if constexpr (XFORM) {
      if (it + 1 < total) commit(std::integral_constant<int, cur ^ 1>{});
      if (it + 2 < total) issue(std::integral_constant<int, cur>{});
      __builtin_amdgcn_sched_barrier(0);
    } else {
      if (it + NSTAGE - 1 < total) issue(std::integral_constant<int, (cur + NSTAGE - 1) % NSTAGE>{});
    }
    constexpr unsigned stage_off = (unsigned)(cur * STAGE_BYTES);
    float fa[2][TI][4], fb[2][TJ][4];
    auto read_step = [&](auto qc, auto setc) {
      constexpr int q = decltype(qc)::value, set = decltype(setc)::value;
#pragma unroll
      for (int i = 0; i < TI; ++i) {
        lds_frag_f1<(8 * q + 0) * ROWB>(fa[set][i][0], lds_base + stage_off + ioff[i]);
        lds_frag_f1<(8 * q + 1) * ROWB>(fa[set][i][1], lds_base + stage_off + ioff[i]);
        lds_frag_f1<(8 * q + 2) * ROWB>(fa[set][i][2], lds_base + stage_off + ioff[i]);
        lds_frag_f1<(8 * q + 3) * ROWB>(fa[set][i][3], lds_base + stage_off + ioff[i]);
      }
#pragma unroll
      for (int j = 0; j < TJ; ++j) {
        lds_frag_f1<(8 * q + 0) * ROWB>(fb[set][j][0], lds_base + stage_off + joff[j]);
        lds_frag_f1<(8 * q + 1) * ROWB>(fb[set][j][1], lds_base + stage_off + joff[j]);
        lds_frag_f1<(8 * q + 2) * ROWB>(fb[set][j][2], lds_base + stage_off + joff[j]);
        lds_frag_f1<(8 * q + 3) * ROWB>(fb[set][j][3], lds_base + stage_off + joff[j]);
      }
    };
    auto fence = [&](auto setc) {
      constexpr int set = decltype(setc)::value;
      if constexpr (TI == 2)
        MOPOE_DEVICE_ASM("s_waitcnt lgkmcnt(0)" : "+v"(fa[set][0][0]), "+v"(fa[set][0][1]), "+v"(fa[set][0][2]), "+v"(fa[set][0][3]),
                         "+v"(fa[set][1][0]), "+v"(fa[set][1][1]), "+v"(fa[set][1][2]), "+v"(fa[set][1][3]),
                         "+v"(fb[set][0][0]), "+v"(fb[set][0][1]), "+v"(fb[set][0][2]), "+v"(fb[set][0][3]),
                         "+v"(fb[set][1][0]), "+v"(fb[set][1][1]), "+v"(fb[set][1][2]), "+v"(fb[set][1][3]) :: "memory");
      else
        MOPOE_DEVICE_ASM("s_waitcnt lgkmcnt(0)" : "+v"(fa[set][0][0]), "+v"(fa[set][0][1]), "+v"(fa[set][0][2]), "+v"(fa[set][0][3]),
                         "+v"(fb[set][0][0]), "+v"(fb[set][0][1]), "+v"(fb[set][0][2]), "+v"(fb[set][0][3]) :: "memory");
      __builtin_amdgcn_sched_barrier(0);
    };
    auto mfma_step = [&](auto setc) {
      constexpr int set = decltype(setc)::value;
#pragma unroll
      for (int e = 0; e < 4; ++e)
#pragma unroll
        for (int j = 0; j < TJ; ++j)
#pragma unroll
          for (int i = 0; i < TI; ++i)
            acc[i][j] = __builtin_amdgcn_mfma_f32_32x32x2f32(fa[set][i][e], fb[set][j][e], acc[i][j], 0, 0, 0);
    };
    using I0 = std::integral_constant<int, 0>; using I1 = std::integral_constant<int, 1>;
    using I2 = std::integral_constant<int, 2>; using I3 = std::integral_constant<int, 3>;
    if constexpr (EMU != 0) {
      Split3 sa[2][TI], sb[2][TJ];
      auto fence_both = [&]() {
        MOPOE_DEVICE_ASM("s_waitcnt lgkmcnt(0)" ::: "memory");
#pragma unroll
        for (int s = 0; s < 2; ++s)
#pragma unroll
          for (int e = 0; e < 4; ++e) {
#pragma unroll
            for (int i = 0; i < TI; ++i) pin_reg(fa[s][i][e]);
#pragma unroll
            for (int j = 0; j < TJ; ++j) pin_reg(fb[s][j][e]);
          }
        __builtin_amdgcn_sched_barrier(0);
      };
      auto split_pair = [&](auto pc) {
        constexpr int p = decltype(pc)::value;
#pragma unroll
        for (int i = 0; i < TI; ++i) sa[p][i] = split3(fa[0][i], fa[1][i]);
#pragma unroll
        for (int j = 0; j < TJ; ++j) sb[p][j] = split3(fb[0][j], fb[1][j]);
      };
      auto mfma_pair = [&](auto pc) {
        constexpr int p = decltype(pc)::value;
        static_for<6>([&](auto tc) {
#pragma unroll
          for (int j = 0; j < TJ; ++j)
#pragma unroll
            for (int i = 0; i < TI; ++i) mfma_split_term<decltype(tc)::value>(acc[i][j], sa[p][i], sb[p][j]);
        });
      };
      read_step(I0{}, I0{});
      read_step(I1{}, I1{});
      fence_both();
      split_pair(I0{});
      __builtin_amdgcn_sched_barrier(0);
      read_step(I2{}, I0{});
      read_step(I3{}, I1{});
      mfma_pair(I0{});
      __builtin_amdgcn_sched_barrier(0);
      fence_both();
      split_pair(I1{});
      __builtin_amdgcn_sched_barrier(0);
      mfma_pair(I1{});
      __builtin_amdgcn_sched_barrier(0);
    } else {
    read_step(I0{}, I0{});
    fence(I0{});
    read_step(I1{}, I1{});
    mfma_step(I0{});
    fence(I1{});
    read_step(I2{}, I0{});
    mfma_step(I1{});
    fence(I0{});
    read_step(I3{}, I1{});
    mfma_step(I0{});
    fence(I1{});
    mfma_step(I1{});
    __builtin_amdgcn_sched_barrier(0);
    }
  };
  {
    int it = 0;
    while (it < total) {
      chunk(it, std::integral_constant<int, 0>{});
      if (++it >= total) break;
      chunk(it, std::integral_constant<int, 1>{});
      if (++it >= total) break;
      if (NSTAGE >= 3) {
        chunk(it, std::integral_constant<int, 2 % NSTAGE>{});
        if (++it >= total) break;
      }
      if (NSTAGE >= 4) {
        chunk(it, std::integral_constant<int, 3 % NSTAGE>{});
        ++it;
      }
    }
  }

  const int l31 = lane & 31, lhi = lane >> 5;
#pragma unroll
  for (int j = 0; j < TJ; ++j) {
    const int co = j0 + wj * WJ + j * 32 + l31;
    if (co >= a.Cout) continue;
#pragma unroll
    for (int i = 0; i < TI; ++i) {
#pragma unroll
      for (int r = 0; r < 16; ++r) {
        const int cii = i0 + wi * WI + i * 32 + (r & 3) + 8 * (r >> 2) + 4 * lhi;
        if (cii >= a.Cin) continue;
        float* dst = a.dW + ((long)tap * a.Cin + cii) * a.Cout + co;
        if (a.atomic) unsafeAtomicAdd(dst, acc[i][j][r]);
        else *dst = acc[i][j][r];
      }
    }
  }
}
```

### mopoe-mimic_amd/mimic_amd/ops.py

```python
from __future__ import annotations

import ctypes as C
import os
from dataclasses import dataclass
from functools import lru_cache
from typing import Optional, Sequence

import torch

_HERE = os.path.dirname(os.path.abspath(__file__))
LIB_PATH = os.environ.get("MOPOE_HIP_LIB") or os.path.join(os.path.dirname(_HERE), "csrc", "libmopoe_hip.so")
ABI_VERSION = 23

RES_A, RES_B = 2.0, 0.3
BN_EPS = 1e-5
SUBSET_MASKS = (1, 2, 4, 3, 5, 6, 7)


class MopoeHipError(RuntimeError):
    pass


class _Geom(C.Structure):
    _fields_ = [(n, C.c_int32) for n in
                ("N", "Hs", "Ws", "Hb", "Wb", "Cin", "Cout", "kh", "kw", "sh", "sw", "ph", "pw", "transposed")]


class _BnRef(C.Structure):
    _fields_ = [("sums", C.c_void_p), ("gamma", C.c_void_p), ("beta", C.c_void_p), ("rmean", C.c_void_p),
                ("rvar", C.c_void_p), ("inv_count", C.c_double), ("eps", C.c_float), ("C", C.c_int32),
                ("mode", C.c_int32)]


class _MaskRef(C.Structure):
    _fields_ = [("mask", C.c_void_p), ("kind", C.c_int32), ("rows_per_sample", C.c_int32)]


class _MixRef(C.Structure):
    _fields_ = [("s", C.c_void_p), ("bn", _BnRef), ("a", C.c_float), ("b", C.c_float)]


class _RunDesc(C.Structure):
    _fields_ = [("sums", C.c_void_p), ("rmean", C.c_void_p), ("rvar", C.c_void_p), ("C", C.c_int32),
                ("count", C.c_int32)]


class _AdamSeg(C.Structure):
    _fields_ = [("p", C.c_void_p), ("g", C.c_void_p), ("m", C.c_void_p), ("v", C.c_void_p), ("p16", C.c_void_p),
                ("n", C.c_int64)]


@dataclass(frozen=True)
class Geom:
    N: int
    Hs: int
    Ws: int
    Hb: int
    Wb: int
    Cin: int
    Cout: int
    kh: int
    kw: int
    sh: int
    sw: int
    ph: int
    pw: int
    transposed: bool

    def __post_init__(self):
        object.__setattr__(self, "_hash", hash((self.N, self.Hs, self.Ws, self.Hb, self.Wb, self.Cin, self.Cout, self.kh,
                                                self.kw, self.sh, self.sw, self.ph, self.pw, self.transposed)))

    def __hash__(self):
        return self._hash

    @property
    def in_shape(self):
        return (self.N, self.Hs, self.Ws, self.Cin) if self.transposed else (self.N, self.Hb, self.Wb, self.Cin)

    @property
    def out_shape(self):
        return (self.N, self.Hb, self.Wb, self.Cout) if self.transposed else (self.N, self.Hs, self.Ws, self.Cout)

    @property
    def taps(self):
        return self.kh * self.kw

    def with_batch(self, n):
        return _with_batch(self, n)

    def c(self):
        return _geom_struct(self)


@lru_cache(maxsize=None)
def _with_batch(g: "Geom", n: int) -> "Geom":
    return Geom(n, *[getattr(g, f) for f in
                     ("Hs", "Ws", "Hb", "Wb", "Cin", "Cout", "kh", "kw", "sh", "sw", "ph", "pw", "transposed")])


@lru_cache(maxsize=None)
def _geom_struct(g: "Geom") -> "_Geom":
    return _Geom(g.N, g.Hs, g.Ws, g.Hb, g.Wb, g.Cin, g.Cout, g.kh, g.kw, g.sh, g.sw, g.ph, g.pw, int(g.transposed))


@dataclass
class Bn:
    gamma: torch.Tensor
    beta: torch.Tensor
    mode: int
    sums: Optional[torch.Tensor] = None
    count: int = 0
    rmean: Optional[torch.Tensor] = None
    rvar: Optional[torch.Tensor] = None
    eps: float = BN_EPS

    def c(self):
        return _BnRef(_p(self.sums), _p(self.gamma), _p(self.beta), _p(self.rmean), _p(self.rvar),
                      (1.0 / self.count) if self.count else 0.0, self.eps, self.gamma.numel(), self.mode)


@dataclass
class Mask:
    mask: torch.Tensor
    kind: int
    rows_per_sample: int = 1

    def c(self):
        return _MaskRef(_p(self.mask), self.kind, self.rows_per_sample)


_NO_BN = _BnRef(None, None, None, None, None, 0.0, 0.0, 0, 0)
_NO_MASK = _MaskRef(None, 0, 1)


def _p(t: Optional[torch.Tensor]):
    return None if t is None else C.c_void_p(t.data_ptr())


_lib = None


def lib():
    global _lib
    if _lib is None:
        if not os.path.exists(LIB_PATH):
            raise MopoeHipError(f"{LIB_PATH} not built: run `python __graft_entry__.py build` "
                                "(mimic_amd has no CPU fallback)")
        _lib = C.CDLL(LIB_PATH)
        _lib.mopoe_last_error.restype = C.c_char_p
        _lib.mopoe_abi_version.restype = C.c_int
        if _lib.mopoe_abi_version() != ABI_VERSION:
            raise MopoeHipError("libmopoe_hip.so ABI version mismatch")
    return _lib


def _check(rc: int):
    if rc != 0:
        raise MopoeHipError(f"libmopoe_hip error {rc}: {lib().mopoe_last_error().decode()}")


_raw_stream = getattr(torch._C, "_cuda_getCurrentRawStream", None)


def _stream_ptr(device=None) -> int:
# ... 329 lines not shown
        if tile >= 5 and taps * (ck // 64) < 2:
            continue
        cap = _GLDS_TILES[tile] if tile >= 5 else (512 if tile == 3 else 768)
        cands[(tile, 1)] = min(1.0, blocks / cap)
        for sp in _SPLITS:
            if sp * 2 <= iters and blocks * sp <= 2048 and sp * per <= ws_bytes:
                cands[(tile, sp)] = min(1.0, blocks * sp / cap)
    return cands


def conv_mix_supported(x, g: Geom) -> bool:
    return _is16(x) or (g.Cin % 4 == 0 and g.Cout % 4 == 0)


def conv_fwd(x, wp, g: Geom, bn_in: Optional[Bn] = None, bias=None, mask: Optional[Mask] = None,
             out_stats=None, out_dtype=None, mix=None):
    _dev(x, wp, bias, out_stats)
    assert tuple(x.shape) == g.in_shape and tuple(wp.shape) == (g.taps, g.Cin, g.Cout)
    out_dtype = out_dtype or x.dtype
    gc = g.c()
    stream = _stream()
    mixr = None
    if mix is not None:
        ms, mbn = mix[0], mix[1]
        _dev(ms)
        assert tuple(ms.shape) == g.out_shape and ms.dtype == out_dtype and ms.is_contiguous() and conv_mix_supported(x, g)
        mixc = _MixRef(ms.data_ptr(), mbn.c(), float(mix[2]) if len(mix) > 2 else RES_A, float(mix[3]) if len(mix) > 3 else RES_B)
        mixr = C.byref(mixc)
    if _is16(x) or out_dtype == BF16:
        plain = bn_in is None and mask is None
        if not g.transposed and g.Cin == 1:
            assert plain and bias is None and x.dtype == torch.float32 and wp.dtype == torch.float32
            y = torch.empty(g.out_shape, dtype=BF16, device=x.device)
            _check(lib().mopoe_edge_expand_bf16(_p(x), _p(wp), _p(y), C.byref(gc), g.Cout, _p(out_stats), stream))
            return y
        if g.transposed and g.Cout == 1:
            assert plain and out_stats is None and _is16(x) and wp.dtype == torch.float32
            y = torch.empty(g.out_shape, dtype=torch.float32, device=x.device)
            _check(lib().mopoe_edge_reduce_bf16(_p(x), _p(wp), _p(bias), _p(y), C.byref(gc), g.Cin, stream))
            return y
        if not (_is16(x) and _is16(wp)):
            raise MopoeHipError("bf16 conv needs a bf16 activation and the bf16 copy of the packed weight")
        y = torch.empty(g.out_shape, dtype=out_dtype, device=x.device)
        ws, nbytes = _workspace(x.device)
        fn = lib().mopoe_conv_fwd_bf16
        bnr, mr, f32 = _bn(bn_in), _mask(mask), C.c_int32(int(out_dtype == torch.float32))

        def launch16(plan, stats=None):
            if mixr is not None:
                _check(lib().mopoe_conv_fwd_mix_bf16(_p(x), _p(wp), _p(bias), _p(y), C.byref(gc), bnr, mr, mixr, _p(stats),
                                                     plan, _p(ws), C.c_size_t(nbytes), stream))
                return
            _check(fn(_p(x), _p(wp), _p(bias), _p(y), f32, C.byref(gc), bnr, mr, _p(stats), plan, _p(ws),
                      C.c_size_t(nbytes), stream))

        key = ("fwd16", g, bn_in is not None, mask is not None, out_stats is not None, out_dtype) + (("mix",) if mix is not None else ())
        plan = _tuned_plan(key, lambda: _gather_candidates_bf16("fwd", g, nbytes, plain_operand=bn_in is None),
                           lambda ref: launch16(ref, _scratch_like(out_stats)))
        launch16(plan, out_stats)
        return y
    y = torch.empty(g.out_shape, dtype=torch.float32, device=x.device)
    ws, nbytes = _workspace(x.device)
    fn = lib().mopoe_conv_fwd
    bnr, mr = _bn(bn_in), _mask(mask)

    def launch(plan, stats=None):
        if mixr is not None:
            _check(lib().mopoe_conv_fwd_mix(_p(x), _p(wp), _p(bias), _p(y), C.byref(gc), bnr, mr, mixr, _p(stats), plan,
                                            _p(ws), C.c_size_t(nbytes), stream))
            return
        _check(fn(_p(x), _p(wp), _p(bias), _p(y), C.byref(gc), bnr, mr, _p(stats), plan, _p(ws), C.c_size_t(nbytes),
                  stream))

    key = ("fwd", g, bn_in is not None, mask is not None, out_stats is not None) + (("mix",) if mix is not None else ())
    plan = _tuned_plan(key, lambda: _gather_candidates("fwd", g, nbytes, plain_operand=bn_in is None),
                       lambda ref: launch(ref, _scratch_like(out_stats)))
    launch(plan, out_stats)
    return y


def conv_dgrad(dy, wp, g: Geom, relu_bn: Optional[Bn] = None, xin=None, bwd_sums=None, out_dtype=None):
    _dev(dy, wp, xin, bwd_sums)
    assert tuple(dy.shape) == g.out_shape
    out_dtype = out_dtype or dy.dtype
    gc = g.c()
    stream = _stream()
    if _is16(dy) or out_dtype == BF16:
        if g.transposed and g.Cout == 1:
            assert relu_bn is None and dy.dtype == torch.float32 and wp.dtype == torch.float32
            dx = torch.empty(g.in_shape, dtype=BF16, device=dy.device)
            _check(lib().mopoe_edge_expand_bf16(_p(dy), _p(wp), _p(dx), C.byref(gc), g.Cin, None, stream))
            return dx
        if not (_is16(dy) and _is16(wp)) or (xin is not None and not _is16(xin)):
            raise MopoeHipError("bf16 conv_dgrad needs bf16 dy / xin and the bf16 copy of the packed weight")
        dx = torch.empty(g.in_shape, dtype=out_dtype, device=dy.device)
        ws, nbytes = _workspace(dy.device)
        fn = lib().mopoe_conv_dgrad_bf16
        bnr, f32 = _bn(relu_bn), C.c_int32(int(out_dtype == torch.float32))

        def launch16(plan, sums=None):
            _check(fn(_p(dy), _p(wp), _p(dx), f32, C.byref(gc), bnr, _p(xin), _p(sums), plan, _p(ws), C.c_size_t(nbytes),
                      stream))

        key = ("dgrad16", g, relu_bn is not None, bwd_sums is not None, out_dtype)
        plan = _tuned_plan(key, lambda: _gather_candidates_bf16("dgrad", g, nbytes, plain_operand=True),
                           lambda ref: launch16(ref, _scratch_like(bwd_sums)))
        launch16(plan, bwd_sums)
        return dx
    dx = torch.empty(g.in_shape, dtype=torch.float32, device=dy.device)
    ws, nbytes = _workspace(dy.device)
    fn = lib().mopoe_conv_dgrad
    bnr = _bn(relu_bn)

    def launch(plan, sums=None):
        _check(fn(_p(dy), _p(wp), _p(dx), C.byref(gc), bnr, _p(xin), _p(sums), plan, _p(ws), C.c_size_t(nbytes), stream))

    key = ("dgrad", g, relu_bn is not None, bwd_sums is not None)
    plan = _tuned_plan(key, lambda: _gather_candidates("dgrad", g, nbytes, plain_operand=True),
                       lambda ref: launch(ref, _scratch_like(bwd_sums)))
    launch(plan, bwd_sums)
    return dx


def conv_wgrad(x, dy, g: Geom, bn_in: Optional[Bn] = None, out=None):
    _dev(x, dy, out)
    assert tuple(x.shape) == g.in_shape and tuple(dy.shape) == g.out_shape
    dwp = out if out is not None else torch.empty((g.taps, g.Cin, g.Cout), dtype=torch.float32, device=x.device)
    assert tuple(dwp.shape) == (g.taps, g.Cin, g.Cout) and dwp.dtype == torch.float32
    gc = g.c()
    stream = _stream()
    bnr = _bn(bn_in)
    if _is16(x) or _is16(dy):
        if min(g.Cin, g.Cout) == 1:
            assert bn_in is None
            vec, scal = (dy, x) if g.Cin == 1 else (x, dy)
            assert _is16(vec) and scal.dtype == torch.float32
            _check(lib().mopoe_edge_wgrad_bf16(_p(vec), _p(scal), _p(dwp), C.byref(gc), max(g.Cin, g.Cout),
                                               C.c_int32(int(out is not None)), stream))
            return dwp
        if not (_is16(x) and _is16(dy)):
            raise MopoeHipError("bf16 conv_wgrad needs both operands in bf16")
        fn = lib().mopoe_conv_wgrad_bf16
        key = ("wgrad16", g, bn_in is not None)
    else:
        fn = lib().mopoe_conv_wgrad
        key = ("wgrad", g, bn_in is not None)

    def launch(plan, dst, is_zero):
        _check(fn(_p(x), _p(dy), _p(dst), C.byref(gc), bnr, C.c_int32(is_zero), plan, stream))

    plan = _tuned_plan(key, lambda: _wgrad_candidates(g, bf16=key[0] == "wgrad16", plain_operand=bn_in is None),
                       lambda ref: launch(ref, _scratch_like(dwp), 1))
    launch(plan, dwp, int(out is not None))
    return dwp


def _rows(t):
    return t.numel() // t.shape[-1]


def block_out_fwd(s, m, bn_s: Bn, a=RES_A, b=RES_B, out_stats=None):
    _dev(s, m, out_stats)
    out = torch.empty_like(s)
    fn = lib().mopoe_block_out_fwd_bf16 if _is16(s) else lib().mopoe_block_out_fwd
    _check(fn(_p(s), _p(m), _p(out), C.c_int64(_rows(s)), s.shape[-1], _bn(bn_s),
                                     C.c_float(a), C.c_float(b), _p(out_stats), _stream()))
    return out


def bn_relu_apply(x, bn: Bn):
    _dev(x)
    out = torch.empty_like(x)
    fn = lib().mopoe_bn_relu_apply_bf16 if _is16(x) else lib().mopoe_bn_relu_apply
    _check(fn(_p(x), _p(out), C.c_int64(_rows(x)), x.shape[-1], _bn(bn), _stream()))
    return out


BLOCK_FRONT = os.environ.get("MOPOE_BLOCK_FRONT", "1") != "0"
BLOCK_FRONT_F32 = os.environ.get("MOPOE_BLOCK_FRONT_F32", "1") != "0"
BLOCK_FRONT_F32_FWD = os.environ.get("MOPOE_BLOCK_FRONT_F32_FWD", "0") != "0"


def block_front_supported(x, g1: "Geom", mask1: Optional[Mask], forward: bool = False) -> bool:
    if forward and not _is16(x) and not BLOCK_FRONT_F32_FWD:
        return False
    return (BLOCK_FRONT and x.dtype in (BF16, torch.float32) and (_is16(x) or BLOCK_FRONT_F32) and g1.Cin == 64 and g1.Cout == 64
            and g1.taps == 1 and _rows(x) % 32 == 0
            and (mask1 is None or (mask1.kind == 1 and mask1.rows_per_sample % 32 == 0)))


def block_front_stats(x, w1, bias, bn1: Bn, mask1: Optional[Mask], out_stats):
    _dev(x, w1, bias, out_stats)
    fn = lib().mopoe_block_front_stats_bf16 if _is16(x) else lib().mopoe_block_front_stats
    _check(fn(_p(x), _p(w1), _p(bias), C.c_int64(_rows(x)), x.shape[-1], _bn(bn1), _mask(mask1),
                                              _p(out_stats), _stream()))
    return out_stats


def block_front_apply(x, w1, bias, bn1: Bn, bn2: Bn, mask1: Optional[Mask]):
    _dev(x, w1, bias)
    a2 = torch.empty_like(x)
    fn = lib().mopoe_block_front_apply_bf16 if _is16(x) else lib().mopoe_block_front_apply
    _check(fn(_p(x), _p(w1), _p(bias), _p(a2), C.c_int64(_rows(x)), x.shape[-1], _bn(bn1), _bn(bn2),
                                              _mask(mask1), _stream()))
    return a2


def block_front_bwd(x, dh2, w1, bias, bn1: Bn, bn2: Bn, mask1: Optional[Mask], sums2, sums1, dw1, dbias=None, dgamma2=None,
                    dbeta2=None):
    _dev(x, dh2, w1, bias, sums2, sums1, dw1, dbias, dgamma2, dbeta2)
    dh1 = torch.empty_like(x)
    fn = lib().mopoe_block_front_bwd_bf16 if _is16(x) else lib().mopoe_block_front_bwd
    _check(fn(_p(x), _p(dh2), _p(w1), _p(bias), _p(dh1), C.c_int64(_rows(x)), x.shape[-1], _bn(bn1),
                                            _bn(bn2), _mask(mask1), _p(sums2), _p(sums1), _p(dw1), _p(dbias), _p(dgamma2), _p(dbeta2),
                                            _stream()))
    return dh1


def bn_bwd_reduce(g, s, bn_s: Bn, sums=None):
    _dev(g, s, sums)
    if sums is None:
        sums = new_stats(s.shape[-1], s.device)
    fn = lib().mopoe_bn_bwd_reduce_bf16 if _is16(s) else lib().mopoe_bn_bwd_reduce
    _check(fn(_p(g), _p(s), C.c_int64(_rows(s)), s.shape[-1], _bn(bn_s), _p(sums), _stream()))
    return sums


def block_out_bwd(g, s, bn_s: Bn, sums, mask: Optional[Mask], a=RES_A, b=RES_B, want_colsum_dm=False,
                  want_colsum_ds=True, small=None):
    _dev(g, s, sums)
    c = s.shape[-1]
    dm, ds = torch.empty_like(g), torch.empty_like(g)
    if small is None:
        small = torch.zeros(4, c, dtype=torch.float32, device=g.device)
    cdm = small[2] if want_colsum_dm else None
    cds = small[3] if want_colsum_ds else None
    fn = lib().mopoe_block_out_bwd_bf16 if _is16(s) else lib().mopoe_block_out_bwd
    _check(fn(_p(g), _p(s), _p(dm), _p(ds), C.c_int64(_rows(s)), c, _bn(bn_s), _p(sums), _mask(mask), C.c_float(a),
              C.c_float(b), _p(small[0]), _p(small[1]), _p(cdm), _p(cds), _stream()))
    return dm, ds, small[0], small[1], cdm, cds


def bn_bwd_apply(dy, x, bn: Bn, sums, mask: Optional[Mask] = None, add=None, want_colsum=False, small=None,
                 next_s=None, next_bn: Optional[Bn] = None, next_sums=None):
    _dev(dy, x, sums, add, next_s, next_sums)
    c = x.shape[-1]
    dx = torch.empty_like(x)
    if small is None:
        small = torch.zeros(3, c, dtype=torch.float32, device=x.device)
    cs = small[2] if want_colsum else None
    nb = _bn(next_bn) if next_s is not None else None
    fn = lib().mopoe_bn_bwd_apply_bf16 if _is16(x) else lib().mopoe_bn_bwd_apply
    _check(fn(_p(dy), _p(x), _p(add), _p(dx), C.c_int64(_rows(x)), c, _bn(bn), _p(sums), _mask(mask), _p(small[0]),
              _p(small[1]), _p(cs), _p(next_s), nb, _p(next_sums), _stream()))
    return dx, small[0], small[1], cs


def bn_running_update(entries: Sequence, momentum=0.1):
    entries = list(entries)
    if not entries:
        return
    arr = (_RunDesc * len(entries))()
    for i, (sums, rm, rv, count) in enumerate(entries):
        _dev(sums, rm, rv)
        arr[i] = _RunDesc(sums.data_ptr(), rm.data_ptr(), rv.data_ptr(), rm.numel(), count)
    _check(lib().mopoe_bn_running_update(arr, len(entries), C.c_float(momentum), _stream()))


STAMPS = None


def stamp(name):
    st = STAMPS
    if st is None:
        return
    if "buf" not in st:
        st["buf"] = torch.zeros(256, dtype=torch.int64, device="cuda")
        st["names"] = []
    i = len(st["names"])
    if i >= st["buf"].numel():
        return
    st["names"].append(name)
    _check(lib().mopoe_prof_stamp(C.c_void_p(st["buf"].data_ptr() + 8 * i), _stream()))


def adam_step(params, grads, ms, vs, step, lr, beta1, beta2, eps, coef, lowp=None, prep=True):
    n = len(params)
    arr = (_AdamSeg * n)()
    for i in range(n):
        p_, g_ = params[i], grads[i]
        if g_ is None:
            arr[i] = _AdamSeg(p_.data_ptr(), None, ms[i].data_ptr(), vs[i].data_ptr(), None, p_.numel())
            continue
        if g_.dtype != torch.float32 or p_.dtype != torch.float32 or g_.numel() != p_.numel():
            raise MopoeHipError("adam_step: parameters and gradients must be fp32 tensors of equal size")
        _dev(p_, g_, ms[i], vs[i])
        lp = lowp[i] if lowp is not None else None
        arr[i] = _AdamSeg(p_.data_ptr(), g_.data_ptr(), ms[i].data_ptr(), vs[i].data_ptr(),
                          None if lp is None else lp.data_ptr(), p_.numel())
    lr_dev = lr if isinstance(lr, torch.Tensor) else None
    _check(lib().mopoe_adam_step(arr, n, _p(step) if prep else None, _p(lr_dev), C.c_double(0.0 if lr_dev is not None else float(lr)),
                                 C.c_double(beta1), C.c_double(beta2), C.c_double(eps), _p(coef), _stream()))


def colsum(x, out=None):
    _dev(x, out)
    zero = out is not None
# ... 431 lines not shown
```

### mopoe-mimic_amd/mimic_amd/trunk.py

```python
from __future__ import annotations

import os
from dataclasses import dataclass
from typing import Dict, List, Optional

import torch

from . import ops
from .layout import ResBlockParams
from .ops import Bn, Geom, Mask


@dataclass
class BlockSpec:
    params: ResBlockParams
    g1: Geom
    g2: Geom
    twod: bool
    name: str


class MaskSource:

    def __init__(self, replay: Optional[Dict[str, torch.Tensor]] = None, prefix: str = ""):
        self.replay, self.prefix = replay, prefix

    def begin(self, sizes, device):
        self._pool, self._off = None, 0
        if self.replay is None and sizes:
            self._pool = torch.empty(sum(sizes), dtype=torch.float32, device=device).bernoulli_(0.5).mul_(2.0)

    def _take(self, count):
        v = self._pool[self._off:self._off + count]
        self._off += count
        return v

    def get(self, name: str, n: int, rows_per_sample: int, c: int, twod: bool, device) -> Mask:
        if self.replay is None and getattr(self, "_pool", None) is not None:
            if twod:
                return Mask(self._take(n * c).view(n, c), 1, rows_per_sample)
            return Mask(self._take(n * rows_per_sample * c).view(n, rows_per_sample, c), 2, rows_per_sample)
        if self.replay is not None:
            m = self.replay[self.prefix + name].to(device=device, dtype=torch.float32)
            if twod:
                return Mask(m.reshape(n, c).contiguous(), 1, rows_per_sample)
            return Mask(m.reshape(n, c, rows_per_sample).permute(0, 2, 1).contiguous(), 2, rows_per_sample)
        if twod:
            m = (torch.rand(n, c, device=device) < 0.5).to(torch.float32).mul_(2.0)
            return Mask(m, 1, rows_per_sample)
        m = (torch.rand(n, rows_per_sample, c, device=device) < 0.5).to(torch.float32).mul_(2.0)
        return Mask(m, 2, rows_per_sample)


WGRAD_SIDE_STREAM = os.environ.get("MOPOE_WGRAD_STREAM", "1") != "0"
FUSE_MIX = os.environ.get("MOPOE_FUSE_MIX", "1") != "0"
FUSE_NEXT_REDUCE = os.environ.get("MOPOE_FUSE_NEXT_REDUCE", "1") != "0"
LANES = os.environ.get("MOPOE_LANES", "0,1").split(",")
LANES_IN_CAPTURE = os.environ.get("MOPOE_LANES_IN_CAPTURE", "0") != "0"
INLINE_LANES_IN_CAPTURE = [x for x in os.environ.get("MOPOE_INLINE_LANES_IN_CAPTURE", "").split(",") if x]
_side_streams = {}


def _side_stream(device, which=0, main=None):
    key = (device.index if device.index is not None else torch.cuda.current_device(), which,
           0 if main is None else main.cuda_stream)
    if key not in _side_streams:
        _side_streams[key] = torch.cuda.Stream(device=device)
    return _side_streams[key]


class _WgradLane:

    def __init__(self, device, which=0):
        self.enabled = (WGRAD_SIDE_STREAM and device.type == "cuda" and str(which) in LANES
                        and (LANES_IN_CAPTURE or not torch.cuda.is_current_stream_capturing()))
        if (not self.enabled and INLINE_LANES_IN_CAPTURE and WGRAD_SIDE_STREAM and device.type == "cuda"
                and str(which) in INLINE_LANES_IN_CAPTURE and torch.cuda.is_current_stream_capturing()):
            from .lanes import _net_streams
            cur = torch.cuda.current_stream(device)
            self.enabled = all(cur.cuda_stream != s.cuda_stream for s in _net_streams.values())
        if self.enabled:
            self.main = torch.cuda.current_stream(device)
            self.side = _side_stream(device, which, self.main)
        self.keep = []

    def run(self, fn, *inputs):
        if not self.enabled:
            return fn()
        ev = torch.cuda.Event()
        ev.record(self.main)
        self.keep.extend(inputs)
        with torch.cuda.stream(self.side):
            self.side.wait_event(ev)
            return fn()

    def join(self):
        if self.enabled:
            self.main.wait_stream(self.side)
        self.keep.clear()


def _bn(p, training: bool, sums, count) -> Bn:
    if training:
        return Bn(p.weight, p.bias, 1, sums=sums, count=count)
    return Bn(p.weight, p.bias, 2, rmean=p.running_mean, rvar=p.running_var)


def stats_needed(blocks: List[BlockSpec]) -> int:
    n = 2 * blocks[0].g1.Cin
    for b in blocks:
        n += 2 * (b.g1.Cin + 2 * b.g2.Cout)
    return n


class StatsArena:

    def __init__(self, n_doubles: int, device, enabled: bool):
        self.buf = torch.zeros(n_doubles, dtype=torch.float64, device=device) if enabled else None
        self.off = 0

    def take(self, c: int):
        if self.buf is None:
            return None
        v = self.buf[self.off:self.off + 2 * c].view(2, c)
        self.off += 2 * c
        return v


MATERIALIZE = os.environ.get("MOPOE_MATERIALIZE", "1")


def _materialize(g2, d1) -> bool:
    return MATERIALIZE != "0"


def _master_weight(mod):
    return mod.weight


def trunk_forward(blocks: List[BlockSpec], x, x_stats, training: bool, dropout: bool, masks: MaskSource,
                  arena: StatsArena, batch: int, wsel=_master_weight):
    saved = []
    running = []
    lane = _WgradLane(x.device, 1)
    if dropout:
        sizes = []
        for spec in blocks:
            rin = spec.g1.Hs * spec.g1.Ws
            rout = spec.g2.Hb * spec.g2.Wb if spec.g2.transposed else spec.g2.Hs * spec.g2.Ws
            sizes += [batch * spec.g1.Cout * (1 if spec.twod else rin), batch * spec.g2.Cout * (1 if spec.twod else rout)]
        masks.begin(sizes, x.device)
    for spec in blocks:
        p, g1, g2 = spec.params, spec.g1.with_batch(batch), spec.g2.with_batch(batch)
        rows_in = x.numel() // x.shape[-1]
        rps_in = rows_in // batch
        bn1 = _bn(p.bn1, training, x_stats, rows_in)
        if training:
            running.append((x_stats, p.bn1, rows_in))
        mask1 = mask2 = None
        if dropout:
            mask1 = masks.get(spec.name + ".dropout1", batch, rps_in, g1.Cout, spec.twod, x.device)
        st_d1 = arena.take(g1.Cout)
        st_s = arena.take(g2.Cout)
        sconv, sbn = p.short[0], p.short[1]
        s = lane.run(lambda: ops.conv_fwd(x, wsel(sconv), g2, bias=sconv.bias, out_stats=st_s), x)
        front_bwd = _materialize(g2, x) and ops.block_front_supported(x, g1, mask1)
        front = _materialize(g2, x) and ops.block_front_supported(x, g1, mask1, forward=True)
        if front:
            if training:
                ops.block_front_stats(x, wsel(p.conv1), p.conv1.bias, bn1, mask1, st_d1)
            d1 = None
        else:
            d1 = ops.conv_fwd(x, wsel(p.conv1), g1, bn_in=bn1, bias=p.conv1.bias, mask=mask1, out_stats=st_d1)
        bn2 = _bn(p.bn2, training, st_d1, rows_in)
        if training:
            running.append((st_d1, p.bn2, rows_in))
        rows_out = batch * (g2.Hb * g2.Wb if g2.transposed else g2.Hs * g2.Ws)
        rps_out = rows_out // batch
        if dropout:
            mask2 = masks.get(spec.name + ".dropout2", batch, rps_out, g2.Cout, spec.twod, x.device)
        lane.join()
        bns = _bn(sbn, training, st_s, rows_out)
        if training:
            running.append((st_s, sbn, rows_out))
        st_out = arena.take(g2.Cout)
        if front:
            a2 = ops.block_front_apply(x, wsel(p.conv1), p.conv1.bias, bn1, bn2, mask1)
        else:
            a2 = ops.bn_relu_apply(d1, bn2) if _materialize(g2, d1) else None
        op2, bn_in2 = (d1, bn2) if a2 is None else (a2, None)
        if FUSE_MIX and ops.conv_mix_supported(x, g2):
            out = ops.conv_fwd(op2, wsel(p.conv2), g2, bn_in=bn_in2, bias=p.conv2.bias, mask=mask2, mix=(s, bns), out_stats=st_out)
        else:
            m = ops.conv_fwd(op2, wsel(p.conv2), g2, bn_in=bn_in2, bias=p.conv2.bias, mask=mask2)
            out = ops.block_out_fwd(s, m, bns, out_stats=st_out)
        saved.append(dict(x=x, d1=d1, a2=a2, s=s, bn1=bn1, bn2=bn2, bns=bns, mask1=mask1, mask2=mask2, g1=g1, g2=g2,
                          front_bwd=front_bwd or front))
        x, x_stats = out, st_out
    return x, saved, running


class BackwardArena:

    def __init__(self, blocks: List["BlockSpec"], device, extra: int = 0):
        nd = sum(2 * b.g2.Cout + 4 * b.g1.Cin for b in blocks)
        nf = sum(4 * b.g2.Cout + 6 * b.g1.Cin for b in blocks)
        nw = sum(b.g1.taps * b.g1.Cin * b.g1.Cout + 2 * b.g2.taps * b.g2.Cin * b.g2.Cout for b in blocks)
        extra = (extra + 3) // 4 * 4 + 64 + 48 * len(blocks)
        raw = torch.zeros(nd * 8 + (nf + nw + extra) * 4, dtype=torch.uint8, device=device)
        self.dbuf = raw[:nd * 8].view(torch.float64)
        self.fbuf = raw[nd * 8:].view(torch.float32)
        self.off = [0, 0]

    def take_w(self, geom):
        return self.take_misc((geom.taps, geom.Cin, geom.Cout))

    def take_d(self, c):
        v = self.dbuf[self.off[0]:self.off[0] + 2 * c].view(2, c)
        self.off[0] += 2 * c
        return v

    def take_f(self, k, c):
        return self.take_misc((k, c))

    def take_misc(self, shape):
        n = 1
        for d in shape:
            n *= int(d)
        start = (self.off[1] + 3) // 4 * 4
        if start + n > self.fbuf.numel():
            return torch.zeros(tuple(shape), dtype=torch.float32, device=self.fbuf.device)
        self.off[1] = start + n
        return self.fbuf[start:start + n].view(tuple(shape))


def trunk_backward(blocks: List[BlockSpec], saved, g, grads: Dict[str, torch.Tensor], wsel=_master_weight,
                   arena: Optional[BackwardArena] = None):
    ar = arena if arena is not None else BackwardArena(blocks, g.device)
    take_w, take_d, take_f, fbuf = ar.take_w, ar.take_d, ar.take_f, ar.fbuf

    lane = _WgradLane(g.device, 0)
    lane_s = _WgradLane(g.device, 1)
    order = list(zip(reversed(blocks), reversed(saved)))
    sums_s = None
    for bi, (spec, sv) in enumerate(order):
        p, g1, g2 = spec.params, sv["g1"], sv["g2"]
        x, d1, s = sv["x"], sv["d1"], sv["s"]
        bn1, bn2, bns = sv["bn1"], sv["bn2"], sv["bns"]
        has_bias = p.conv1.bias is not None
        n = spec.name
        if sums_s is None:
            sums_s = ops.bn_bwd_reduce(g, s, bns, sums=take_d(g2.Cout))
        dm, ds, dgs, dbs, cdm, cds = ops.block_out_bwd(g, s, bns, sums_s, sv["mask2"],
                                                       want_colsum_dm=has_bias, want_colsum_ds=True,
                                                       small=take_f(4, g2.Cout))
        sums2 = take_d(g1.Cout)
        a2 = sv.get("a2")
        front = bool(sv.get("front_bwd"))
        if d1 is None:
            bn2y = Bn(bn2.gamma, bn2.beta, 3, sums=bn2.sums, count=bn2.count, eps=bn2.eps)
            dh2 = ops.conv_dgrad(dm, wsel(p.conv2), g2, relu_bn=bn2y, xin=a2, bwd_sums=sums2)
        else:
            dh2 = ops.conv_dgrad(dm, wsel(p.conv2), g2, relu_bn=bn2, xin=d1, bwd_sums=sums2)
        w2, ws_ = take_w(g2), take_w(g2)
        if a2 is None:
            grads[f"{n}.conv2.weight"] = lane.run(lambda: ops.conv_wgrad(d1, dm, g2, bn_in=bn2, out=w2), d1, dm)
        else:
            grads[f"{n}.conv2.weight"] = lane.run(lambda: ops.conv_wgrad(a2, dm, g2, out=w2), a2, dm)
        grads[f"{n}.{p.short_name}.0.weight"] = lane.run(lambda: ops.conv_wgrad(x, ds, g2, out=ws_), x, ds)
        dxs = lane_s.run(lambda: ops.conv_dgrad(ds, wsel(p.short[0]), g2), ds)
        grads[f"{n}.{p.short_name}.0.bias"] = cds
        grads[f"{n}.{p.short_name}.1.weight"] = dgs
        grads[f"{n}.{p.short_name}.1.bias"] = dbs
        if front:
            small = take_f(3, g1.Cin)
            sums1 = take_d(g1.Cin)
            w1 = take_w(g1)
            dh1 = ops.block_front_bwd(x, dh2, wsel(p.conv1), p.conv1.bias, bn1, bn2, sv["mask1"], sums2, sums1, w1,
                                      dbias=small[2] if has_bias else None, dgamma2=small[0], dbeta2=small[1])
            grads[f"{n}.bn2.weight"], grads[f"{n}.bn2.bias"] = small[0], small[1]
            grads[f"{n}.conv1.weight"] = w1
            cdc1 = small[2]
        else:
            dc1, dg2, db2, cdc1 = ops.bn_bwd_apply(dh2, d1, bn2, sums2, mask=sv["mask1"], want_colsum=has_bias,
                                                   small=take_f(3, g1.Cin))
            grads[f"{n}.bn2.weight"], grads[f"{n}.bn2.bias"] = dg2, db2
            sums1 = take_d(g1.Cin)
            dh1 = ops.conv_dgrad(dc1, wsel(p.conv1), g1, relu_bn=bn1, xin=x, bwd_sums=sums1)
            w1 = take_w(g1)
            grads[f"{n}.conv1.weight"] = lane.run(lambda: ops.conv_wgrad(x, dc1, g1, bn_in=bn1, out=w1), x, dc1)
        if has_bias:
            grads[f"{n}.conv2.bias"] = cdm
            grads[f"{n}.conv1.bias"] = cdc1
        lane_s.join()
        nxt = order[bi + 1][1] if bi + 1 < len(order) else None
        if nxt is not None and FUSE_NEXT_REDUCE:
            sums_s = take_d(g1.Cin)
            g, dg1, db1, _ = ops.bn_bwd_apply(dh1, x, bn1, sums1, add=dxs, small=take_f(3, g1.Cin),
                                              next_s=nxt["s"], next_bn=nxt["bns"], next_sums=sums_s)
        else:
            sums_s = None
            g, dg1, db1, _ = ops.bn_bwd_apply(dh1, x, bn1, sums1, add=dxs, small=take_f(3, g1.Cin))
        grads[f"{n}.bn1.weight"], grads[f"{n}.bn1.bias"] = dg1, db1
    lane.join()
    return g, fbuf


def apply_running_updates(running, momentum=0.1):
    if not running:
        return
    ops.bn_running_update([(sums, bn.running_mean, bn.running_var, count) for sums, bn, count in running],
                          momentum)
    for _, bn, _ in running:
        bn.pending_batches += 1
```

Baseline: 6667 samples/sec.

## Batch deferred weight-gradient convolutions into grouped multi-member kernel launches

Weight-gradient convolutions in the trunk backward are deferred and collected, then launched as grouped kernels. Each grouped kernel holds up to 16 members in its argument table and maps each block to a member by prefix offsets. This cuts the number of small kernel launches and lets small wgrad GEMMs share one grid for better device fill. In exchange the wgrads run later, at the end of the backward on the side lane, which delays their overlap with other work and keeps activations alive longer, capped by a byte budget.

Result: no change. 6641 samples/sec (-0.4%).

```diff
diff --git a/include/mopoe_hip.h b/include/mopoe_hip.h
--- a/include/mopoe_hip.h
+++ b/include/mopoe_hip.h
@@ -8,7 +8,7 @@
 extern "C" {
 #endif
 
-#define MOPOE_ABI_VERSION 23
+#define MOPOE_ABI_VERSION 24
 
 #define MOPOE_OK 0
 #define MOPOE_ERR_ARG (-1)
diff --git a/include/mopoe_hip_group.h b/include/mopoe_hip_group.h
--- /dev/null
+++ b/include/mopoe_hip_group.h
@@ -0,0 +1,29 @@
+#ifndef MOPOE_HIP_GROUP_H
+#define MOPOE_HIP_GROUP_H
+
+#include "mopoe_hip.h"
+
+#ifdef __cplusplus
+extern "C" {
+#endif
+
+#define MOPOE_WGRAD_GROUP_MAX 16
+
+typedef struct {
+  const float* x;
+  const float* dy;
+  float* dwp;
+  mopoe_conv_geom geom;
+  const mopoe_bn_ref* bn_in;
+  int32_t dwp_is_zero;
+  const mopoe_conv_plan* plan;
+} mopoe_conv_wgrad_member;
+
+int mopoe_conv_wgrad_group_class(const mopoe_conv_wgrad_member* m);
+
+int mopoe_conv_wgrad_group(const mopoe_conv_wgrad_member* m, int32_t n, void* stream);
+
+#ifdef __cplusplus
+}
+#endif
+#endif
diff --git a/mopoe-mimic_amd/csrc/conv_gemm.hip b/mopoe-mimic_amd/csrc/conv_gemm.hip
--- a/mopoe-mimic_amd/csrc/conv_gemm.hip
+++ b/mopoe-mimic_amd/csrc/conv_gemm.hip
@@ -1,4 +1,5 @@
 #include "gemm_common.hpp"
+#include "../../include/mopoe_hip_group.h"
 
 namespace mopoe {
 
@@ -664,7 +665,8 @@
 };
 
 template <int BI, int BJ, bool VEC, int SPEC = 0>
-__global__ __launch_bounds__(256) void wgrad_gemm_kernel(const WgradArgs a) {
+__device__ __forceinline__ void wgrad_gemm_body(const WgradArgs& a, const unsigned lin0, const unsigned gx, const unsigned gy,
+                                                const unsigned gz) {
   static_assert(SPEC == 0 || VEC, "specialised loops exist for the vector path only");
   constexpr int WI = BI / 2, WJ = BJ / 2;
   constexpr int TI = WI / 32, TJ = WJ / 32;
@@ -680,11 +682,9 @@
   const int tid = threadIdx.x;
   const int lane = tid & 63, wave = tid >> 6;
   const int wi = wave >> 1, wj = wave & 1;
-  const unsigned lin = a.xcd_remap ? xcd_swizzle(blockIdx.x + gridDim.x * (blockIdx.y + gridDim.y * blockIdx.z),
-                                                 gridDim.x * gridDim.y * gridDim.z)
-                                   : blockIdx.x + gridDim.x * (blockIdx.y + gridDim.y * blockIdx.z);
-  const unsigned bx = lin % gridDim.x, byz = lin / gridDim.x;
-  const unsigned by = byz % gridDim.y, bz = byz / gridDim.y;
+  const unsigned lin = a.xcd_remap ? xcd_swizzle(lin0, gx * gy * gz) : lin0;
+  const unsigned bx = lin % gx, byz = lin / gx;
+  const unsigned by = byz % gy, bz = byz / gy;
   const int it_i = bx / a.nJ, it_j = bx % a.nJ;
   const int i0 = it_i * BI, j0 = it_j * BJ;
   const int tap = by;
@@ -912,6 +912,33 @@
       }
     }
   }
+}
+
+template <int BI, int BJ, bool VEC, int SPEC = 0>
+__global__ __launch_bounds__(256) void wgrad_gemm_kernel(const WgradArgs a) {
+  wgrad_gemm_body<BI, BJ, VEC, SPEC>(a, blockIdx.x + gridDim.x * (blockIdx.y + gridDim.y * blockIdx.z), gridDim.x, gridDim.y, gridDim.z);
+}
+
+constexpr int WGRAD_GROUP_MAX = MOPOE_WGRAD_GROUP_MAX;
+struct WgradGroupArgs {
+  WgradArgs m[WGRAD_GROUP_MAX];
+  unsigned first[WGRAD_GROUP_MAX + 1];
+  unsigned gx[WGRAD_GROUP_MAX], gy[WGRAD_GROUP_MAX];
+  int n;
+};
+static_assert(sizeof(WgradGroupArgs) <= 4096, "the group table must fit the kernel argument segment");
+
+__device__ __forceinline__ int wgrad_group_member(const WgradGroupArgs& g, unsigned b) {
+  int i = 0;
+  while (i + 1 < g.n && b >= g.first[i + 1]) ++i;
+  return __builtin_amdgcn_readfirstlane(i);
+}
+
+template <int BI, int BJ, bool VEC, int SPEC = 0>
+__global__ __launch_bounds__(256) void wgrad_gemm_group_kernel(const WgradGroupArgs g) {
+  const int i = wgrad_group_member(g, blockIdx.x);
+  const unsigned cnt = g.first[i + 1] - g.first[i];
+  wgrad_gemm_body<BI, BJ, VEC, SPEC>(g.m[i], blockIdx.x - g.first[i], g.gx[i], g.gy[i], cnt / (g.gx[i] * g.gy[i]));
 }
 
 #ifndef EPI_MAX_BLOCKS_Y
@@ -1201,22 +1228,37 @@
                        nullptr, relu_bn, xin, bwd_sums, plan, workspace, workspace_bytes, (hipStream_t)stream);
 }
 
-extern "C" int mopoe_conv_wgrad(const float* x, const float* dy, float* dwp, const mopoe_conv_geom* g,
-                                const mopoe_bn_ref* bn_in, int32_t dwp_is_zero, const mopoe_conv_plan* plan,
-                                void* stream_) {
+enum { WG_GLDS_EMU = 0,
+       WG_GLDS = 2,
+       WG_VEC = 6,
+       WG_SCALAR = 12,
+       WG_NINST = 14,
+       WG_EDGE_DY = -1, WG_EDGE_X = -2, WG_PARITY = -3 };
+
+struct WgradLaunch {
+  WgradArgs a;
+  int inst;
+  dim3 grid;
+  bool vec;
+  size_t xb, db;
+  size_t dw_bytes;
+  double flops, abytes;
+  int prof_kind;
+};
+
+static int wgrad_prepare(const float* x, const float* dy, float* dwp, const mopoe_conv_geom* g, const mopoe_bn_ref* bn_in,
+                         const mopoe_conv_plan* plan, WgradLaunch* L) {
   if (int rc = validate_geom(g)) return rc;
   if (!x || !dy || !dwp) { set_error("conv_wgrad: null pointer"); return MOPOE_ERR_ARG; }
-  hipStream_t stream = (hipStream_t)stream_;
-  if ((!bn_in || bn_in->mode == 0) && !g->transposed && g->Cin == 1 && edge_supported(g, g->Cout, {dy, dwp}))
-    return edge_wgrad(dy, x, dwp, g, g->Cout, stream, dwp_is_zero != 0);
-  if ((!bn_in || bn_in->mode == 0) && g->transposed && g->Cout == 1 && edge_supported(g, g->Cin, {x, dwp}))
-    return edge_wgrad(x, dy, dwp, g, g->Cin, stream, dwp_is_zero != 0);
-  WgradArgs a;
+  if ((!bn_in || bn_in->mode == 0) && !g->transposed && g->Cin == 1 && edge_supported(g, g->Cout, {dy, dwp})) { L->inst = WG_EDGE_DY; return MOPOE_OK; }
+  if ((!bn_in || bn_in->mode == 0) && g->transposed && g->Cout == 1 && edge_supported(g, g->Cin, {x, dwp})) { L->inst = WG_EDGE_X; return MOPOE_OK; }
+  WgradArgs& a = L->a;
   a.Xs = x; a.Dy = dy; a.dW = dwp;
   a.N = g->N; a.Hs = g->Hs; a.Ws = g->Ws; a.Hb = g->Hb; a.Wb = g->Wb; a.Cin = g->Cin; a.Cout = g->Cout;
   a.kh = g->kh; a.kw = g->kw; a.sh = g->sh; a.sw = g->sw; a.ph = g->ph; a.pw = g->pw;
   a.x_is_big = g->transposed ? 0 : 1;
   a.Ms = (long)g->N * g->Hs * g->Ws;
+  a.chunk = 0; a.nJ = 0; a.atomic = 0; a.xcd_remap = 0;
   mopoe_bn_ref none = {};
   a.bn_in = bn_in ? *bn_in : none;
   if (a.bn_in.mode != 0 && (a.bn_in.C != g->Cin || g->Cin > MAX_BN_C)) { set_error("wgrad bn_in channel mismatch"); return MOPOE_ERR_ARG; }
@@ -1226,44 +1268,16 @@
   const size_t rows_dy = (size_t)g->N * (g->transposed ? g->Hb * g->Wb : g->Hs * g->Ws);
   const size_t xb = rows_x * g->Cin * sizeof(float), db = rows_dy * g->Cout * sizeof(float);
   const bool vec = a.vecI && a.vecJ && xb < (1ull << 31) && db < (1ull << 31);
+  L->vec = vec; L->xb = xb; L->db = db;
   a.x_bytes = (unsigned)std::min<size_t>(xb, 0x7fffffffu);
   a.dy_bytes = (unsigned)std::min<size_t>(db, 0x7fffffffu);
   if (rows_x >= (1ull << 31) || rows_dy >= (1ull << 31)) { set_error("wgrad: more than 2^31 rows"); return MOPOE_ERR_ARG; }
   const int hw_s = g->Hs * g->Ws;
   a.fast = (vec && ((g->Ws % BK == 0) || (BK % g->Ws == 0 && hw_s % BK == 0))) ? 1 : 0;
   const int taps = g->kh * g->kw;
+  L->dw_bytes = (size_t)taps * g->Cin * g->Cout * sizeof(float);
   bool big = g->Cin > 64 && g->Cout > 64;
-  if (plan && (plan->tile == 9 || plan->tile == 10)) {
-    const bool ok = a.bn_in.mode == 0 && vec && g->kh == 4 && g->kw == 4 && g->sh == 2 && g->sw == 2 && g->ph == 1 && g->pw == 1 &&
-                    g->Hs % 8 == 0 && g->Ws % 8 == 0 && g->Hb == 2 * g->Hs && g->Wb == 2 * g->Ws;
-    if (!ok) {
-      set_error("wgrad plan: tiles 9 / 10 (four taps per block) need a plain operand, the vector path, k4 s2 p1 and a small grid of whole 8 x 8 tiles");
-      return MOPOE_ERR_ARG;
-    }
-    const int Cg = a.x_is_big ? g->Cin : g->Cout, Csm = a.x_is_big ? g->Cout : g->Cin;
-    const int cs = plan->tile == 10 ? 128 : 64;
-    if (cs == 128 && Csm % 128 != 0) { set_error("wgrad plan: tile 10 needs a multiple of 128 channels on the small-grid operand (%d)", Csm); return MOPOE_ERR_ARG; }
-    const long ntiles = (long)g->N * (g->Hs / 8) * (g->Ws / 8);
-    const long cblocks = (long)ceil_div(Cg, 64) * ceil_div(Csm, cs) * 4;
-    long split = plan->split > 0 ? plan->split : (256 + cblocks - 1) / cblocks;
-    if (split > ntiles) split = ntiles;
-    if (split < 1) split = 1;
-    a.chunk = (ntiles + split - 1) / split;
-    split = (ntiles + a.chunk - 1) / a.chunk;
-    a.atomic = split > 1;
-    static const bool xcd_remap9 = !getenv("MOPOE_NO_XCD_REMAP");
-    a.xcd_remap = xcd_remap9 ? 1 : 0;
-    if (a.atomic && !dwp_is_zero) {
-      if (hipMemsetAsync(dwp, 0, (size_t)taps * g->Cin * g->Cout * sizeof(float), stream) != hipSuccess) { set_error("wgrad memset failed"); return MOPOE_ERR_LAUNCH; }
-    }
-    ProfScope prof(stream, 2.0 * (double)a.Ms * g->Cin * (double)g->Cout * taps, PROF_F32_WGRAD_PARITY + (cs == 128 ? 2 : 0) + (a.x_is_big ? 0 : 1), (double)xb + (double)db);
-    const dim3 grid((unsigned)(ceil_div(Cg, 64) * ceil_div(Csm, cs)), 4, (unsigned)split);
-    if (cs == 128 && a.x_is_big) hipLaunchKernelGGL((wgrad_parity_f32_kernel<128, true>), grid, dim3(256), 0, stream, a);
-    else if (cs == 128) hipLaunchKernelGGL((wgrad_parity_f32_kernel<128, false>), grid, dim3(256), 0, stream, a);
-    else if (a.x_is_big) hipLaunchKernelGGL((wgrad_parity_f32_kernel<64, true>), grid, dim3(256), 0, stream, a);
-    else hipLaunchKernelGGL((wgrad_parity_f32_kernel<64, false>), grid, dim3(256), 0, stream, a);
-    return check_launch("wgrad_parity_f32 (four taps per block)");
-  }
+  if (plan && (plan->tile == 9 || plan->tile == 10)) { L->inst = WG_PARITY; return MOPOE_OK; }
   const bool wemu = plan && (plan->tile == 7 || plan->tile == 8);
   if (wemu && a.bn_in.mode != 0) { set_error("wgrad plan: tile %d (split-bf16 products) has no BN-on-load form", plan->tile); return MOPOE_ERR_ARG; }
   if (plan && (plan->tile == 2 || plan->tile == 6 || plan->tile == 8)) big = false;
@@ -1290,43 +1304,138 @@
   a.atomic = split > 1;
   static const bool xcd_remap = !getenv("MOPOE_NO_XCD_REMAP");
   a.xcd_remap = xcd_remap ? 1 : 0;
-  const size_t bytes = (size_t)taps * g->Cin * g->Cout * sizeof(float);
+  L->flops = 2.0 * (double)a.Ms * g->Cin * (double)g->Cout * taps;
+  const int spec = a.fast ? (a.bn_in.mode != 0 ? 2 : 1) : 0;
+  L->abytes = ((double)g->N * g->Hs * g->Ws * (g->transposed ? g->Cin : g->Cout)
+               + (double)g->N * g->Hb * g->Wb * (g->transposed ? g->Cout : g->Cin)) * sizeof(float);
+  L->prof_kind = wemu ? PROF_F32_WGRAD_GLDS_EMU + (big ? 0 : 1)
+                 : glds ? PROF_F32_WGRAD_GLDS + (big ? 0 : 2) + (a.bn_in.mode != 0 ? 1 : 0)
+                        : (vec ? PROF_WGRAD_VEC + (big ? 0 : 3) + spec : PROF_WGRAD_SCALAR + (big ? 0 : 1));
+  L->inst = wemu ? WG_GLDS_EMU + (big ? 0 : 1)
+            : glds ? WG_GLDS + (big ? 0 : 2) + (a.bn_in.mode != 0 ? 1 : 0)
+                   : (vec ? WG_VEC + (big ? 0 : 3) + spec : WG_SCALAR + (big ? 0 : 1));
+  L->grid = dim3(nI * nJ, taps, (unsigned)split);
+  return MOPOE_OK;
+}
+
+typedef void (*WgradKernel)(const WgradArgs);
+typedef void (*WgradGroupKernel)(const WgradGroupArgs);
+struct WgradKernels { WgradKernel one; WgradGroupKernel group; };
+#define WG_GLDS_PAIR(...) WgradKernels{wgrad_gemm_f32_glds_kernel<__VA_ARGS__>, wgrad_gemm_f32_glds_group_kernel<__VA_ARGS__>}
+#define WG_GEMM_PAIR(...) WgradKernels{wgrad_gemm_kernel<__VA_ARGS__>, wgrad_gemm_group_kernel<__VA_ARGS__>}
+static WgradKernels wgrad_kernels(int inst) {
+  switch (inst) {
+    case WG_GLDS_EMU + 0: return WG_GLDS_PAIR(128, false, 2, 1);
+    case WG_GLDS_EMU + 1: return WG_GLDS_PAIR(64, false, 4, 1);
+    case WG_GLDS + 0: return WG_GLDS_PAIR(128, false, 2);
+    case WG_GLDS + 1: return WG_GLDS_PAIR(128, true, 2);
+    case WG_GLDS + 2: return WG_GLDS_PAIR(64, false, 4);
+    case WG_GLDS + 3: return WG_GLDS_PAIR(64, true, 2);
+    case WG_VEC + 0: return WG_GEMM_PAIR(128, 128, true, 0);
+    case WG_VEC + 1: return WG_GEMM_PAIR(128, 128, true, 1);
+    case WG_VEC + 2: return WG_GEMM_PAIR(128, 128, true, 2);
+    case WG_VEC + 3: return WG_GEMM_PAIR(64, 64, true, 0);
+    case WG_VEC + 4: return WG_GEMM_PAIR(64, 64, true, 1);
+    case WG_VEC + 5: return WG_GEMM_PAIR(64, 64, true, 2);
+    case WG_SCALAR + 0: return WG_GEMM_PAIR(128, 128, false);
+    default: return WG_GEMM_PAIR(64, 64, false);
+  }
+}
+#undef WG_GLDS_PAIR
+#undef WG_GEMM_PAIR
+
+extern "C" int mopoe_conv_wgrad(const float* x, const float* dy, float* dwp, const mopoe_conv_geom* g,
+                                const mopoe_bn_ref* bn_in, int32_t dwp_is_zero, const mopoe_conv_plan* plan,
+                                void* stream_) {
+  WgradLaunch L;
+  if (int rc = wgrad_prepare(x, dy, dwp, g, bn_in, plan, &L)) return rc;
+  hipStream_t stream = (hipStream_t)stream_;
+  if (L.inst == WG_EDGE_DY) return edge_wgrad(dy, x, dwp, g, g->Cout, stream, dwp_is_zero != 0);
+  if (L.inst == WG_EDGE_X) return edge_wgrad(x, dy, dwp, g, g->Cin, stream, dwp_is_zero != 0);
+  WgradArgs& a = L.a;
+  if (L.inst == WG_PARITY) {
+    const int taps = g->kh * g->kw;
+    const bool ok = a.bn_in.mode == 0 && L.vec && g->kh == 4 && g->kw == 4 && g->sh == 2 && g->sw == 2 && g->ph == 1 && g->pw == 1 &&
+                    g->Hs % 8 == 0 && g->Ws % 8 == 0 && g->Hb == 2 * g->Hs && g->Wb == 2 * g->Ws;
+    if (!ok) {
+      set_error("wgrad plan: tiles 9 / 10 (four taps per block) need a plain operand, the vector path, k4 s2 p1 and a small grid of whole 8 x 8 tiles");
+      return MOPOE_ERR_ARG;
+    }
+    const int Cg = a.x_is_big ? g->Cin : g->Cout, Csm = a.x_is_big ? g->Cout : g->Cin;
+    const int cs = plan->tile == 10 ? 128 : 64;
+    if (cs == 128 && Csm % 128 != 0) { set_error("wgrad plan: tile 10 needs a multiple of 128 channels on the small-grid operand (%d)", Csm); return MOPOE_ERR_ARG; }
+    const long ntiles = (long)g->N * (g->Hs / 8) * (g->Ws / 8);
+    const long cblocks = (long)ceil_div(Cg, 64) * ceil_div(Csm, cs) * 4;
+    long split = plan->split > 0 ? plan->split : (256 + cblocks - 1) / cblocks;
+    if (split > ntiles) split = ntiles;
+    if (split < 1) split = 1;
+    a.chunk = (ntiles + split - 1) / split;
+    split = (ntiles + a.chunk - 1) / a.chunk;
+    a.atomic = split > 1;
+    static const bool xcd_remap9 = !getenv("MOPOE_NO_XCD_REMAP");
+    a.xcd_remap = xcd_remap9 ? 1 : 0;
+    if (a.atomic && !dwp_is_zero) {
+      if (hipMemsetAsync(dwp, 0, (size_t)taps * g->Cin * g->Cout * sizeof(float), stream) != hipSuccess) { set_error("wgrad memset failed"); return MOPOE_ERR_LAUNCH; }
+    }
+    ProfScope prof(stream, 2.0 * (double)a.Ms * g->Cin * (double)g->Cout * taps, PROF_F32_WGRAD_PARITY + (cs == 128 ? 2 : 0) + (a.x_is_big ? 0 : 1), (double)L.xb + (double)L.db);
+    const dim3 grid((unsigned)(ceil_div(Cg, 64) * ceil_div(Csm, cs)), 4, (unsigned)split);
+    if (cs == 128 && a.x_is_big) hipLaunchKernelGGL((wgrad_parity_f32_kernel<128, true>), grid, dim3(256), 0, stream, a);
+    else if (cs == 128) hipLaunchKernelGGL((wgrad_parity_f32_kernel<128, false>), grid, dim3(256), 0, stream, a);
+    else if (a.x_is_big) hipLaunchKernelGGL((wgrad_parity_f32_kernel<64, true>), grid, dim3(256), 0, stream, a);
+    else hipLaunchKernelGGL((wgrad_parity_f32_kernel<64, false>), grid, dim3(256), 0, stream, a);
+    return check_launch("wgrad_parity_f32 (four taps per block)");
+  }
   if (a.atomic && !dwp_is_zero) {
-    if (hipMemsetAsync(dwp, 0, bytes, stream) != hipSuccess) { set_error("wgrad memset failed"); return MOPOE_ERR_LAUNCH; }
-  }
-  const double flops = 2.0 * (double)a.Ms * g->Cin * (double)g->Cout * taps;
-  const int spec = a.fast ? (a.bn_in.mode != 0 ? 2 : 1) : 0;
-  const double abytes = ((double)g->N * g->Hs * g->Ws * (g->transposed ? g->Cin : g->Cout)
-                         + (double)g->N * g->Hb * g->Wb * (g->transposed ? g->Cout : g->Cin)) * sizeof(float);
-  ProfScope prof(stream, flops, wemu ? PROF_F32_WGRAD_GLDS_EMU + (big ? 0 : 1)
-                                : glds ? PROF_F32_WGRAD_GLDS + (big ? 0 : 2) + (a.bn_in.mode != 0 ? 1 : 0)
-                                     : (vec ? PROF_WGRAD_VEC + (big ? 0 : 3) + spec : PROF_WGRAD_SCALAR + (big ? 0 : 1)), abytes);
-  dim3 grid(nI * nJ, taps, (unsigned)split);
-  if (wemu) {
-    if (big) hipLaunchKernelGGL((wgrad_gemm_f32_glds_kernel<128, false, 2, 1>), grid, dim3(256), 0, stream, a);
-    else hipLaunchKernelGGL((wgrad_gemm_f32_glds_kernel<64, false, 4, 1>), grid, dim3(256), 0, stream, a);
-  } else if (glds) {
-    const bool xf = a.bn_in.mode != 0;
-    if (big) {
-      if (xf) hipLaunchKernelGGL((wgrad_gemm_f32_glds_kernel<128, true, 2>), grid, dim3(256), 0, stream, a);
-      else hipLaunchKernelGGL((wgrad_gemm_f32_glds_kernel<128, false, 2>), grid, dim3(256), 0, stream, a);
-    } else {
-      if (xf) hipLaunchKernelGGL((wgrad_gemm_f32_glds_kernel<64, true, 2>), grid, dim3(256), 0, stream, a);
-      else hipLaunchKernelGGL((wgrad_gemm_f32_glds_kernel<64, false, 4>), grid, dim3(256), 0, stream, a);
-    }
-  } else if (vec) {
-    if (big) {
-      if (spec == 1) hipLaunchKernelGGL((wgrad_gemm_kernel<128, 128, true, 1>), grid, dim3(256), 0, stream, a);
-      else if (spec == 2) hipLaunchKernelGGL((wgrad_gemm_kernel<128, 128, true, 2>), grid, dim3(256), 0, stream, a);
-      else hipLaunchKernelGGL((wgrad_gemm_kernel<128, 128, true, 0>), grid, dim3(256), 0, stream, a);
-    } else {
-      if (spec == 1) hipLaunchKernelGGL((wgrad_gemm_kernel<64, 64, true, 1>), grid, dim3(256), 0, stream, a);
-      else if (spec == 2) hipLaunchKernelGGL((wgrad_gemm_kernel<64, 64, true, 2>), grid, dim3(256), 0, stream, a);
-      else hipLaunchKernelGGL((wgrad_gemm_kernel<64, 64, true, 0>), grid, dim3(256), 0, stream, a);
-    }
-  } else {
-    if (big) hipLaunchKernelGGL((wgrad_gemm_kernel<128, 128, false>), grid, dim3(256), 0, stream, a);
-    else hipLaunchKernelGGL((wgrad_gemm_kernel<64, 64, false>), grid, dim3(256), 0, stream, a);
-  }
+    if (hipMemsetAsync(dwp, 0, L.dw_bytes, stream) != hipSuccess) { set_error("wgrad memset failed"); return MOPOE_ERR_LAUNCH; }
+  }
+  ProfScope prof(stream, L.flops, L.prof_kind, L.abytes);
+  hipLaunchKernelGGL(wgrad_kernels(L.inst).one, L.grid, dim3(256), 0, stream, a);
   return check_launch("wgrad_gemm");
 }
+
+static int wgrad_prepare_member(const mopoe_conv_wgrad_member* m, WgradLaunch* L) {
+  if (!m) { set_error("conv_wgrad_group: null member"); return MOPOE_ERR_ARG; }
+  if (int rc = wgrad_prepare(m->x, m->dy, m->dwp, &m->geom, m->bn_in, m->plan, L)) return rc;
+  if (L->inst == WG_PARITY) { set_error("conv_wgrad_group: plan tiles 9 / 10 (four taps per block) do not group"); return MOPOE_ERR_ARG; }
+  if (L->inst < 0) { set_error("conv_wgrad_group: a single-channel layer runs on the streaming edge kernels, which do not group"); return MOPOE_ERR_ARG; }
+  return MOPOE_OK;
+}
+
+extern "C" int mopoe_conv_wgrad_group_class(const mopoe_conv_wgrad_member* m) {
+  WgradLaunch L;
+  if (int rc = wgrad_prepare_member(m, &L)) return rc;
+  return L.inst;
+}
+
+extern "C" int mopoe_conv_wgrad_group(const mopoe_conv_wgrad_member* m, int32_t n, void* stream_) {
+  if (!m || n < 2 || n > WGRAD_GROUP_MAX) { set_error("conv_wgrad_group: 2 to %d members (%d)", WGRAD_GROUP_MAX, (int)n); return MOPOE_ERR_ARG; }
+  hipStream_t stream = (hipStream_t)stream_;
+  WgradGroupArgs ga;
+  ga.n = n;
+  int inst = -1, prof_kind = 0;
+  double flops = 0.0, abytes = 0.0;
+  unsigned long long blocks = 0;
+  for (int i = 0; i < n; ++i) {
+    WgradLaunch L;
+    if (int rc = wgrad_prepare_member(&m[i], &L)) return rc;
+    if (i == 0) { inst = L.inst; prof_kind = L.prof_kind; }
+    else if (L.inst != inst) { set_error("conv_wgrad_group: member %d is another kernel instantiation (%d) than member 0 (%d)", i, L.inst, inst); return MOPOE_ERR_ARG; }
+    ga.m[i] = L.a;
+    ga.first[i] = (unsigned)blocks;
+    ga.gx[i] = L.grid.x; ga.gy[i] = L.grid.y;
+    blocks += (unsigned long long)L.grid.x * L.grid.y * L.grid.z;
+    flops += L.flops; abytes += L.abytes;
+  }
+  if (blocks >= (1ull << 31)) { set_error("conv_wgrad_group: more than 2^31 blocks"); return MOPOE_ERR_ARG; }
+  for (int i = n; i < WGRAD_GROUP_MAX; ++i) { ga.m[i] = ga.m[0]; ga.gx[i] = ga.gy[i] = 1; }
+  for (int i = n; i <= WGRAD_GROUP_MAX; ++i) ga.first[i] = (unsigned)blocks;
+  for (int i = 0; i < n; ++i) {
+    if (ga.m[i].atomic && !m[i].dwp_is_zero) {
+      const size_t bytes = (size_t)m[i].geom.kh * m[i].geom.kw * m[i].geom.Cin * m[i].geom.Cout * sizeof(float);
+      if (hipMemsetAsync(m[i].dwp, 0, bytes, stream) != hipSuccess) { set_error("wgrad memset failed"); return MOPOE_ERR_LAUNCH; }
+    }
+  }
+  ProfScope prof(stream, flops, prof_kind, abytes);
+  hipLaunchKernelGGL(wgrad_kernels(inst).group, dim3((unsigned)blocks), dim3(256), 0, stream, ga);
+  return check_launch("wgrad_gemm (grouped)");
+}
diff --git a/mopoe-mimic_amd/csrc/conv_gemm_glds.inc b/mopoe-mimic_amd/csrc/conv_gemm_glds.inc
--- a/mopoe-mimic_amd/csrc/conv_gemm_glds.inc
+++ b/mopoe-mimic_amd/csrc/conv_gemm_glds.inc
@@ -454,7 +454,8 @@
 }
 
 template <int BI, bool XFORM, int NSTAGE, int EMU = 0>
-__global__ __launch_bounds__(256, 2) void wgrad_gemm_f32_glds_kernel(const WgradArgs a) {
+__device__ __forceinline__ void wgrad_gemm_f32_glds_body(const WgradArgs& a, const unsigned lin0, const unsigned gx, const unsigned gy,
+                                                         const unsigned gz) {
   static_assert(EMU == 0 || !XFORM, "EMU: plain operand form");
   constexpr int BJ = BI;
   constexpr int WI = BI / 2, WJ = BJ / 2, TI = WI / 32, TJ = WJ / 32;
@@ -476,11 +477,9 @@
   const int tid = threadIdx.x;
   const int lane = tid & 63, wave = __builtin_amdgcn_readfirstlane(tid >> 6);
   const int wi = wave >> 1, wj = wave & 1;
-  const unsigned lin = a.xcd_remap ? xcd_swizzle(blockIdx.x + gridDim.x * (blockIdx.y + gridDim.y * blockIdx.z),
-                                                 gridDim.x * gridDim.y * gridDim.z)
-                                   : blockIdx.x + gridDim.x * (blockIdx.y + gridDim.y * blockIdx.z);
-  const unsigned bx = lin % gridDim.x, byz = lin / gridDim.x;
-  const unsigned by = byz % gridDim.y, bz = byz / gridDim.y;
+  const unsigned lin = a.xcd_remap ? xcd_swizzle(lin0, gx * gy * gz) : lin0;
+  const unsigned bx = lin % gx, byz = lin / gx;
+  const unsigned by = byz % gy, bz = byz / gy;
   const int it_i = bx / a.nJ, it_j = bx % a.nJ;
   const int i0 = it_i * BI, j0 = it_j * BJ;
   const int tap = by;
@@ -751,3 +750,16 @@
     }
   }
 }
+
+template <int BI, bool XFORM, int NSTAGE, int EMU = 0>
+__global__ __launch_bounds__(256, 2) void wgrad_gemm_f32_glds_kernel(const WgradArgs a) {
+  wgrad_gemm_f32_glds_body<BI, XFORM, NSTAGE, EMU>(a, blockIdx.x + gridDim.x * (blockIdx.y + gridDim.y * blockIdx.z), gridDim.x, gridDim.y,
+                                                   gridDim.z);
+}
+
+template <int BI, bool XFORM, int NSTAGE, int EMU = 0>
+__global__ __launch_bounds__(256, 2) void wgrad_gemm_f32_glds_group_kernel(const WgradGroupArgs g) {
+  const int i = wgrad_group_member(g, blockIdx.x);
+  const unsigned cnt = g.first[i + 1] - g.first[i];
+  wgrad_gemm_f32_glds_body<BI, XFORM, NSTAGE, EMU>(g.m[i], blockIdx.x - g.first[i], g.gx[i], g.gy[i], cnt / (g.gx[i] * g.gy[i]));
+}
diff --git a/mopoe-mimic_amd/mimic_amd/ops.py b/mopoe-mimic_amd/mimic_amd/ops.py
--- a/mopoe-mimic_amd/mimic_amd/ops.py
+++ b/mopoe-mimic_amd/mimic_amd/ops.py
@@ -10,7 +10,7 @@
 
 _HERE = os.path.dirname(os.path.abspath(__file__))
 LIB_PATH = os.environ.get("MOPOE_HIP_LIB") or os.path.join(os.path.dirname(_HERE), "csrc", "libmopoe_hip.so")
-ABI_VERSION = 23
+ABI_VERSION = 24
 
 RES_A, RES_B = 2.0, 0.3
 BN_EPS = 1e-5
@@ -646,7 +646,98 @@
     plan = _tuned_plan(key, lambda: _wgrad_candidates(g, bf16=key[0] == "wgrad16", plain_operand=bn_in is None),
                        lambda ref: launch(ref, _scratch_like(dwp), 1))
     launch(plan, dwp, int(out is not None))
+    if wgrad_launch_log is not None:
+        wgrad_launch_log.append(("single", (dwp.data_ptr(),)))
     return dwp
+
+
+WGRAD_GROUP = os.environ.get("MOPOE_WGRAD_GROUP", "1") != "0"
+WGRAD_GROUP_MAX = 16
+wgrad_launch_log = None
+
+
+class _WgradMember(C.Structure):
+    _fields_ = [("x", C.c_void_p), ("dy", C.c_void_p), ("dwp", C.c_void_p), ("geom", _Geom), ("bn_in", C.POINTER(_BnRef)),
+                ("dwp_is_zero", C.c_int32), ("plan", C.POINTER(_Plan))]
+
+
+def wgrad_group_chunks(classes, limit=WGRAD_GROUP_MAX):
+    by_class, out = {}, []
+    for i, c in enumerate(classes):
+        if c < 0:
+            out.append([i])
+        else:
+            by_class.setdefault(c, []).append(i)
+    for idx in by_class.values():
+        parts = -(-len(idx) // limit)
+        size = -(-len(idx) // parts)
+        out.extend(idx[k:k + size] for k in range(0, len(idx), size))
+    return out
+
+
+def _wgrad_plan(x, dy, g: Geom, bn_in: Optional[Bn]):
+    def launch(ref):
+        k = (torch.float32, g.taps * g.Cin * g.Cout, x.device)
+        if k not in _scratch:
+            _scratch[k] = torch.zeros(k[1], dtype=torch.float32, device=x.device)
+        dst = _scratch[k]
+        _check(lib().mopoe_conv_wgrad(_p(x), _p(dy), _p(dst), C.byref(g.c()), _bn(bn_in), C.c_int32(1), ref, _stream()))
+
+    return _tuned_plan(("wgrad", g, bn_in is not None), lambda: _wgrad_candidates(g, plain_operand=bn_in is None), launch)
+
+
+def wgrad_deferrable(x, dy, g: Geom, bn_in: Optional[Bn] = None) -> bool:
+    if not WGRAD_GROUP or x.dtype != torch.float32 or dy.dtype != torch.float32:
+        return False
+    if not (x.is_cuda and dy.is_cuda):
+        return True
+    if min(g.Cin, g.Cout) == 1:
+        return False
+    plan = _wgrad_plan(x, dy, g, bn_in)
+    return plan is None or plan._obj.tile not in (9, 10)
+
+
+def _wgrad_group_native(members):
+    if not WGRAD_GROUP or len(members) < 2:
+        return False
+    for x, dy, g, bn_in, out in members:
+        if not (x.is_cuda and dy.is_cuda) or x.dtype != torch.float32 or dy.dtype != torch.float32:
+            return False
+    return True
+
+
+def conv_wgrad_group(members):
+    members = list(members)
+    if not _wgrad_group_native(members):
+        return [conv_wgrad(x, dy, g, bn_in=bn_in, out=out) for x, dy, g, bn_in, out in members]
+    L = lib()
+    stream = _stream()
+    recs, keep, classes, dwps = [], [], [], []
+    for x, dy, g, bn_in, out in members:
+        _dev(x, dy, out)
+        assert tuple(x.shape) == g.in_shape and tuple(dy.shape) == g.out_shape
+        dwp = out if out is not None else torch.empty((g.taps, g.Cin, g.Cout), dtype=torch.float32, device=x.device)
+        assert tuple(dwp.shape) == (g.taps, g.Cin, g.Cout) and dwp.dtype == torch.float32
+        bnc = bn_in.c() if bn_in is not None else None
+        plan = _wgrad_plan(x, dy, g, bn_in)
+        rec = _WgradMember(x.data_ptr(), dy.data_ptr(), dwp.data_ptr(), g.c(), C.pointer(bnc) if bnc is not None else None,
+                           int(out is not None), C.cast(plan, C.POINTER(_Plan)) if plan is not None else None)
+        keep.append((bnc, plan))
+        recs.append(rec)
+        dwps.append(dwp)
+        classes.append(int(L.mopoe_conv_wgrad_group_class(C.byref(rec))))
+    for idx in wgrad_group_chunks(classes):
+        if len(idx) < 2:
+            x, dy, g, bn_in, out = members[idx[0]]
+            got = conv_wgrad(x, dy, g, bn_in=bn_in, out=dwps[idx[0]] if out is not None else None)
+            if out is None:
+                dwps[idx[0]] = got
+            continue
+        arr = (_WgradMember * len(idx))(*[recs[i] for i in idx])
+        _check(L.mopoe_conv_wgrad_group(arr, C.c_int32(len(idx)), stream))
+        if wgrad_launch_log is not None:
+            wgrad_launch_log.append(("group", tuple(dwps[i].data_ptr() for i in idx)))
+    return dwps
 
 
 def _rows(t):
diff --git a/mopoe-mimic_amd/mimic_amd/trunk.py b/mopoe-mimic_amd/mimic_amd/trunk.py
--- a/mopoe-mimic_amd/mimic_amd/trunk.py
+++ b/mopoe-mimic_amd/mimic_amd/trunk.py
@@ -98,6 +98,31 @@
         if self.enabled:
             self.main.wait_stream(self.side)
         self.keep.clear()
+
+
+WGRAD_DEFER_BYTES = int(os.environ.get("MOPOE_WGRAD_DEFER_MB", "96")) << 20
+
+
+class _DeferredWgrads:
+
+    def __init__(self):
+        self.members, self.names, self.bytes = [], [], 0
+
+    def add(self, grads, name, x, dy, g, bn_in, out) -> bool:
+        nbytes = x.numel() * x.element_size() + dy.numel() * dy.element_size()
+        if self.bytes + nbytes > WGRAD_DEFER_BYTES or not ops.wgrad_deferrable(x, dy, g, bn_in):
+            return False
+        self.bytes += nbytes
+        self.members.append((x, dy, g, bn_in, out))
+        self.names.append(name)
+        grads[name] = out
+        return True
+
+    def launch(self, grads):
+        if self.members:
+            for name, dwp in zip(self.names, ops.conv_wgrad_group(self.members)):
+                grads[name] = dwp
+        self.members, self.names, self.bytes = [], [], 0
 
 
 def _bn(p, training: bool, sums, count) -> Bn:
@@ -241,6 +266,7 @@
 
     lane = _WgradLane(g.device, 0)
     lane_s = _WgradLane(g.device, 1)
+    deferred = _DeferredWgrads()
     order = list(zip(reversed(blocks), reversed(saved)))
     sums_s = None
     for bi, (spec, sv) in enumerate(order):
@@ -263,11 +289,11 @@
         else:
             dh2 = ops.conv_dgrad(dm, wsel(p.conv2), g2, relu_bn=bn2, xin=d1, bwd_sums=sums2)
         w2, ws_ = take_w(g2), take_w(g2)
-        if a2 is None:
-            grads[f"{n}.conv2.weight"] = lane.run(lambda: ops.conv_wgrad(d1, dm, g2, bn_in=bn2, out=w2), d1, dm)
-        else:
-            grads[f"{n}.conv2.weight"] = lane.run(lambda: ops.conv_wgrad(a2, dm, g2, out=w2), a2, dm)
-        grads[f"{n}.{p.short_name}.0.weight"] = lane.run(lambda: ops.conv_wgrad(x, ds, g2, out=ws_), x, ds)
+        x2, bn_in2 = (d1, bn2) if a2 is None else (a2, None)
+        if not deferred.add(grads, f"{n}.conv2.weight", x2, dm, g2, bn_in2, w2):
+            grads[f"{n}.conv2.weight"] = lane.run(lambda: ops.conv_wgrad(x2, dm, g2, bn_in=bn_in2, out=w2), x2, dm)
+        if not deferred.add(grads, f"{n}.{p.short_name}.0.weight", x, ds, g2, None, ws_):
+            grads[f"{n}.{p.short_name}.0.weight"] = lane.run(lambda: ops.conv_wgrad(x, ds, g2, out=ws_), x, ds)
         dxs = lane_s.run(lambda: ops.conv_dgrad(ds, wsel(p.short[0]), g2), ds)
         grads[f"{n}.{p.short_name}.0.bias"] = cds
         grads[f"{n}.{p.short_name}.1.weight"] = dgs
@@ -288,7 +314,8 @@
             sums1 = take_d(g1.Cin)
             dh1 = ops.conv_dgrad(dc1, wsel(p.conv1), g1, relu_bn=bn1, xin=x, bwd_sums=sums1)
             w1 = take_w(g1)
-            grads[f"{n}.conv1.weight"] = lane.run(lambda: ops.conv_wgrad(x, dc1, g1, bn_in=bn1, out=w1), x, dc1)
+            if not deferred.add(grads, f"{n}.conv1.weight", x, dc1, g1, bn1, w1):
+                grads[f"{n}.conv1.weight"] = lane.run(lambda: ops.conv_wgrad(x, dc1, g1, bn_in=bn1, out=w1), x, dc1)
         if has_bias:
             grads[f"{n}.conv2.bias"] = cdm
             grads[f"{n}.conv1.bias"] = cdc1
@@ -302,6 +329,8 @@
             sums_s = None
             g, dg1, db1, _ = ops.bn_bwd_apply(dh1, x, bn1, sums1, add=dxs, small=take_f(3, g1.Cin))
         grads[f"{n}.bn1.weight"], grads[f"{n}.bn1.bias"] = dg1, db1
+    if deferred.members:
+        lane.run(lambda: deferred.launch(grads), *[t for m in deferred.members for t in m[:2]])
     lane.join()
     return g, fbuf
 
```
